# hey-yahei/Quantization.MXNet

Hardware: AMD Instinct MI355X
Metric: images/sec int8-sim MobileNet1.0 (per-layer W8A8, online input quant) (higher is better)
Workload: dtype f32

## Files before the change

quantization/mxnet_amd/csrc/fq_core.hip:

```cpp
#include "fq_common.h"

namespace fqi {

thread_local char g_err[512] = "";

int fail(int code, const char* fmt, ...) {
  va_list ap;
  va_start(ap, fmt);
  vsnprintf(g_err, sizeof(g_err), fmt, ap);
  va_end(ap);
  return code;
}

bool g_prof_on = false;
std::mutex g_prof_mu;
std::vector<ProfRec> g_prof;

void prof_push(const ProfRec& r) {
  std::lock_guard<std::mutex> lk(g_prof_mu);
  g_prof.push_back(r);
}

int num_cu() {
  constexpr int kMaxDev = 64;
  static int cache[kMaxDev] = {0};
  int dev = 0;
  if (hipGetDevice(&dev) != hipSuccess || dev < 0 || dev >= kMaxDev) return 256;
  if (cache[dev] == 0) {
    hipDeviceProp_t prop;
    int cu = 0;
    if (hipGetDeviceProperties(&prop, dev) == hipSuccess) cu = prop.multiProcessorCount;
    cache[dev] = cu > 0 ? cu : 256;
  }
  return cache[dev];
}

int max_lds_bytes() {
  constexpr int kMaxDev = 64;
  static int cache[kMaxDev] = {0};
  int dev = 0;
  if (hipGetDevice(&dev) != hipSuccess || dev < 0 || dev >= kMaxDev) return 160 * 1024;
  if (cache[dev] == 0) {
    int v = 0;
    if (hipDeviceGetAttribute(&v, hipDeviceAttributeMaxSharedMemoryPerBlock, dev) != hipSuccess || v <= 0) v = 160 * 1024;
    cache[dev] = v;
  }
  return cache[dev];
}

int env_int(const char* name, int dflt) {
  const char* e = getenv(name);
  return (e && *e) ? atoi(e) : dflt;
}

constexpr int kPolNtLoad_ = 1, kPolNtStore_ = 2, kPolReverse_ = 4;
int stream_policy(int kernel_id, int64_t numel) {
  static const int ov_stat = env_int("FQ_POLICY_STAT", -1);
  static const int ov_on = env_int("FQ_POLICY_ONLINE", -1);
  static const int ov_off = env_int("FQ_POLICY_OFFLINE", -1);
  static const int64_t big = (int64_t)env_int("FQ_POLICY_BIG_MB", 160) * 1000000;
  const bool is_big = numel * (int64_t)sizeof(float) >= big;
  switch (kernel_id) {
    case FQ_KERNEL_STAT:
      return ov_stat >= 0 ? ov_stat : 0;
    case FQ_KERNEL_APPLY_ONLINE:
      if (ov_on >= 0) return ov_on;
      return is_big ? (kPolReverse_ | kPolNtLoad_ | kPolNtStore_) : kPolReverse_;
    default:
      if (ov_off >= 0) return ov_off;
      return is_big ? (kPolNtLoad_ | kPolNtStore_) : 0;
  }
}

}

using namespace fqi;

extern "C" {

const char* fq_last_error(void) { return g_err; }
int fq_version(void) { return 102; }
#ifndef FQ_BUILD_ID
#define FQ_BUILD_ID "0000000000000000000000000000000000000000"
#endif
const char* fq_build_id(void) {
  static const char id[] = "FQ_BUILD_ID=" FQ_BUILD_ID;
  return id + 12;
}

int fq_device_info(char* arch, int arch_len, int* compute_units, int* wavefront) {
  int dev = 0;
  FQ_HIP(hipGetDevice(&dev));
  hipDeviceProp_t prop;
  FQ_HIP(hipGetDeviceProperties(&prop, dev));
  if (arch != nullptr && arch_len > 0) {
    strncpy(arch, prop.gcnArchName, (size_t)arch_len - 1);
    arch[arch_len - 1] = 0;
  }
  if (compute_units) *compute_units = prop.multiProcessorCount;
  if (wavefront) *wavefront = prop.warpSize;
  return FQ_OK;
}

int fq_profile_enable(int on) {
  g_prof_on = on != 0;
  return FQ_OK;
}

int fq_profile_reset(void) {
  std::lock_guard<std::mutex> lk(g_prof_mu);
  for (auto& r : g_prof) {
    (void)hipEventDestroy(r.a);
    (void)hipEventDestroy(r.b);
  }
  g_prof.clear();
  return FQ_OK;
}

int fq_profile_read_moved(int kernel_id, double* total_moved_bytes) {
  FQ_REQUIRE(kernel_id >= 0 && kernel_id < FQ_KERNEL_COUNT, "fq_profile_read_moved: bad kernel id %d", kernel_id);
  FQ_REQUIRE(total_moved_bytes, "fq_profile_read_moved: null pointer");
  std::lock_guard<std::mutex> lk(g_prof_mu);
  double moved = 0.0;
  for (auto& r : g_prof)
    if (r.kid == kernel_id) moved += r.moved;
  *total_moved_bytes = moved;
  return FQ_OK;
}

int fq_profile_read(int kernel_id, double* total_ms, int64_t* launches, double* total_bytes) {
  FQ_REQUIRE(kernel_id >= 0 && kernel_id < FQ_KERNEL_COUNT, "fq_profile_read: bad kernel id %d", kernel_id);
  FQ_REQUIRE(total_ms && launches && total_bytes, "fq_profile_read: null pointer");
  std::lock_guard<std::mutex> lk(g_prof_mu);
  double ms = 0.0, bytes = 0.0;
  int64_t cnt = 0;
  for (auto& r : g_prof) {
    if (r.kid != kernel_id) continue;
    FQ_HIP(hipEventSynchronize(r.b));
    float t = 0.f;
    FQ_HIP(hipEventElapsedTime(&t, r.a, r.b));
    ms += t;
    bytes += r.bytes;
    ++cnt;
  }
  *total_ms = ms;
  *launches = cnt;
  *total_bytes = bytes;
  return FQ_OK;
}

}

namespace {
__global__ void spin_kernel(unsigned long long* __restrict__ t, unsigned long long ticks) {
  const unsigned long long t0 = wall_clock64();
  unsigned long long t1 = t0;
  while (t1 - t0 < ticks) t1 = wall_clock64();
  if (threadIdx.x == 0) {
    t[0] = t0;
    t[1] = t1;
  }
}
}

extern "C" {

int fq_profile_calibrate(void* scratch, int repeats, double* pair_ms, double* null_kernel_ms, fqStream_t stream) {
  FQ_REQUIRE(scratch && pair_ms && null_kernel_ms && repeats > 0 && repeats <= 4096, "fq_profile_calibrate: bad arguments");
  hipStream_t st = (hipStream_t)stream;
  std::vector<hipEvent_t> ev((size_t)repeats * 2 + 2);
  for (auto& e : ev) FQ_HIP(hipEventCreate(&e));
  for (int i = 0; i < repeats; ++i) {
    FQ_HIP(hipEventRecord(ev[2 * i], st));
    hipLaunchKernelGGL(fill_kernel, dim3(1), dim3(64), 0, st, (float*)scratch, (int64_t)1, 0.0f);
    FQ_HIP(hipEventRecord(ev[2 * i + 1], st));
  }
  FQ_HIP(hipEventRecord(ev[2 * repeats], st));
  for (int i = 0; i < repeats; ++i)
    hipLaunchKernelGGL(fill_kernel, dim3(1), dim3(64), 0, st, (float*)scratch, (int64_t)1, 0.0f);
  FQ_HIP(hipEventRecord(ev[2 * repeats + 1], st));
  FQ_HIP(hipEventSynchronize(ev.back()));
  std::vector<float> ts;
  for (int i = 0; i < repeats; ++i) {
    float t = 0.f;
    FQ_HIP(hipEventElapsedTime(&t, ev[2 * i], ev[2 * i + 1]));
    ts.push_back(t);
  }
  float all = 0.f;
  FQ_HIP(hipEventElapsedTime(&all, ev[2 * repeats], ev[2 * repeats + 1]));
  for (auto& e : ev) (void)hipEventDestroy(e);
  std::sort(ts.begin(), ts.end());
  *pair_ms = ts[ts.size() / 2];
  *null_kernel_ms = (double)all / repeats;
  return FQ_OK;
}

int fq_profile_launch_overhead(void* scratch, int repeats, double spin_us, double* overhead_ms, double* spin_ms,
                               fqStream_t stream) {
  FQ_REQUIRE(scratch && overhead_ms && spin_ms && repeats > 0 && repeats <= 4096 && spin_us > 0 && spin_us < 1e5,
             "fq_profile_launch_overhead: bad arguments");
  hipStream_t st = (hipStream_t)stream;
  int dev = 0, khz = 0;
  FQ_HIP(hipGetDevice(&dev));
  FQ_HIP(hipDeviceGetAttribute(&khz, hipDeviceAttributeWallClockRate, dev));
  FQ_REQUIRE(khz > 0, "fq_profile_launch_overhead: the device reports no wall clock rate");
  const unsigned long long ticks = (unsigned long long)(spin_us * 1e-3 * khz);
  std::vector<hipEvent_t> ev((size_t)repeats * 2 + 2);
  for (auto& e : ev) FQ_HIP(hipEventCreate(&e));
  unsigned long long* t = (unsigned long long*)scratch;
  for (int i = 0; i < repeats; ++i) {
    FQ_HIP(hipEventRecord(ev[2 * i], st));
    hipLaunchKernelGGL(spin_kernel, dim3(1), dim3(64), 0, st, t + 2 * i, ticks);
    FQ_HIP(hipEventRecord(ev[2 * i + 1], st));
  }
  FQ_HIP(hipEventRecord(ev[2 * repeats], st));
  for (int i = 0; i < repeats; ++i) hipLaunchKernelGGL(spin_kernel, dim3(1), dim3(64), 0, st, t + 2 * i, ticks);
  FQ_HIP(hipEventRecord(ev[2 * repeats + 1], st));
  FQ_LAUNCH_CHECK();
  FQ_HIP(hipStreamSynchronize(st));
  std::vector<unsigned long long> host((size_t)repeats * 2);
  FQ_HIP(hipMemcpy(host.data(), t, host.size() * sizeof(unsigned long long), hipMemcpyDeviceToHost));
  std::vector<double> pair, own;
  for (int i = 0; i < repeats; ++i) {
    float el = 0.f;
    FQ_HIP(hipEventElapsedTime(&el, ev[2 * i], ev[2 * i + 1]));
    pair.push_back((double)el);
    own.push_back((double)(host[2 * i + 1] - host[2 * i]) / (double)khz);
  }
  float all = 0.f;
  FQ_HIP(hipEventElapsedTime(&all, ev[2 * repeats], ev[2 * repeats + 1]));
  for (auto& e : ev) (void)hipEventDestroy(e);
  std::sort(pair.begin(), pair.end());
  std::sort(own.begin(), own.end());
  *overhead_ms = pair[pair.size() / 2] - (double)all / repeats;
  *spin_ms = own[own.size() / 2];
  return FQ_OK;
}

}
```

quantization/mxnet_amd/csrc/fq_front_layout.h:

```cpp
#pragma once

#include <cstddef>
#include <cstdint>

#if defined(__HIPCC__)
#define FQ_FL_FN __host__ __device__ __forceinline__
#else
#define FQ_FL_FN inline
#endif

namespace fqi {

constexpr int kFrontRows = 8;
constexpr int kFrontBandBytes = 32768;
constexpr int kStatLdsPerCU = 160 * 1024, kStatLdsMax = 120 * 1024;

struct FrontLayout {
  int js;
  int pl;
};

FQ_FL_FN FrontLayout front_layout(int q, int rows) {
  FrontLayout l;
  l.js = rows * q + ((8 - rows * q) & 15);
  l.pl = 4 * l.js + 16;
  return l;
}

FQ_FL_FN int front_slot(FrontLayout l, int p) { return (p & 3) * l.js + (p >> 2); }

FQ_FL_FN int front_byte(FrontLayout l, int c, int p) { return (((c >> 2) * l.pl + front_slot(l, p)) << 2) + (c & 3); }

inline size_t front_band_bytes(int q, int rows, int cin) { return (size_t)((cin + 3) / 4) * front_layout(q, rows).pl * 4; }

FQ_FL_FN int front_channel(int c0, int wave, int segs, int seg) { return c0 + wave * segs + seg; }

FQ_FL_FN int mfma_row_pixel(int i32) { return 16 * ((i32 >> 2) & 1) + 4 * (i32 >> 3) + (i32 & 3); }

inline int stat_wg_per_cu(size_t lds, int cap) {
  const int by_lds = (int)((size_t)kStatLdsPerCU / (lds + 1024));
  return by_lds > cap ? cap : (by_lds < 1 ? 1 : by_lds);
}

inline int front_rows_pick(int64_t n, int64_t h, int64_t w, int cin, size_t lds_fixed, int num_cu, int wg_cap, int forced = 0) {
  const int q = (int)(w / 4);
  int rmax = (int)(kFrontBandBytes / (32 * w));
  rmax = rmax > kFrontRows ? kFrontRows : rmax;
  rmax = rmax > h ? (int)h : rmax;
  while (rmax >= 1 && lds_fixed + front_band_bytes(q, rmax, cin) > (size_t)kStatLdsMax) --rmax;
  if (rmax < 1) return 0;
  if (forced > 0) return forced < rmax ? forced : rmax;
  {
    int r2 = rmax;
    while (r2 >= 1 && stat_wg_per_cu(lds_fixed + front_band_bytes(q, r2, cin), wg_cap) < 2) --r2;
    if (r2 >= 1) rmax = r2;
  }
  double best = 1e30;
  int best_r = rmax;
  bool best_whole = false;
  for (int r = rmax; r >= 1; --r) {
    const int64_t wgs = n * ((h + r - 1) / r);
    const int64_t slots = (int64_t)num_cu * stat_wg_per_cu(lds_fixed + front_band_bytes(q, r, cin), wg_cap);
    const int64_t grid = wgs < slots ? wgs : slots, rounds = (wgs + grid - 1) / grid;
    const double cost = (double)(rounds * ((grid + num_cu - 1) / num_cu) * (r + 2));
    const bool whole = (r * w) % 32 == 0;
    if (cost < best - 1e-9 || (cost < best + 1e-9 && whole && !best_whole)) {
      best = cost;
      best_r = r;
      best_whole = whole;
    }
  }
  return best_r;
}

}
```

quantization/mxnet_amd/csrc/fq_pwdw.hip:

```cpp
#include "fq_pw.h"

#include "fq_front_layout.h"

#include <climits>

namespace {

struct PwDwGeom {
  int Cin, KTS, Cout, H, W, Ho, Wo;
  int strips, ctg, bands, RB;
  int zoff, pitch;
  int vw;
  FastDiv qv;
};

constexpr int kRowSlack = 8;

template <int KT, int S> struct PwDwRing {
  static constexpr int NB = S == 1 ? 2 : (KT <= 2 ? 3 : 4);
  static constexpr int NR = 2;
};

template <int KT, int CW, int S, int LZ, int FAST, int CODES, int NS = 0>
__global__ __launch_bounds__(512) void pwdw_kernel(
// ... 141 lines not shown
      } else {
        return fq_pack4<false>(a, b, c, d, q1, ubias1, nn_xor1);
      }
    };
    constexpr int NO = S == 1 ? 16 : 8;
    float sumA[CW][NO], sumB[S == 1 ? CW : 1][NO];
#pragma unroll
    for (int j = 0; j < CW; ++j)
#pragma unroll
      for (int k = 0; k < NO; ++k) {
        sumA[j][k] = 0.0f;
        if (S == 1) sumB[j][k] = 0.0f;
      }
    QParams qc = q2;
    if (FAST) qc.hi = fminf(q2.hi, top);

    auto row = [&](int t, auto ph_c) __attribute__((always_inline)) {
      constexpr int PH = decltype(ph_c)::value;
      const bool row_ok = t >= 0 && t < g.H;
      v4i afrag[KT];
      if constexpr (CODES) {
        issue_row(t + NR - 1, crow[(PH + NR - 1) % NR]);
        FQ_PIN();
#pragma unroll
        for (int kt = 0; kt < KT; ++kt) afrag[kt] = crow[PH % NR][kt];
      } else {
#pragma unroll
        for (int kt = 0; kt < KT; ++kt) {
          const int qn = kt + NB - 1;
          issue(t + qn / KT, qn % KT, raw[(PH * KT + kt + NB - 1) % NB]);
          FQ_PIN();
          float (&mine)[16] = raw[(PH * KT + kt) % NB];
          v4i f;
#pragma unroll
          for (int d = 0; d < 4; ++d)
            f[d] = pack_x(mine[4 * d + 0], mine[4 * d + 1], mine[4 * d + 2], mine[4 * d + 3]);
          asm volatile("" : "+v"(f[0]), "+v"(f[1]), "+v"(f[2]), "+v"(f[3]));
          afrag[kt] = f;
          FQ_PIN();
        }
      }
      const int r_emit = S == 1 ? t - 1 : (t - 1) >> 1;
      const bool emits = (S == 1 || (t & 1)) && r_emit >= ro0 && r_emit < ro1;
      float* rbuf = rowbuf + (r_emit & 1) * rb_stride;
#pragma unroll
      for (int j = 0; j < CW; ++j) {
        const int ct = cgi * CW + j;
        const float* kc = ldsK + (ct * 32 + i32) * 13;
        auto finish_store = [&](const float (&sum)[NO]) __attribute__((always_inline)) {
          if (!emits) return;
          float* dst = rbuf + (ct * 32 + i32) * g.pitch + obase;
          float mrow = 0.0f;
          const float b2 = kDwLds ? kc[9] : k_b2[j], bsc2 = kDwLds ? kc[10] : k_bsc2[j], bsh2 = kDwLds ? kc[11] : k_bsh2[j];
#pragma unroll
          for (int k = 0; k < NO; ++k) {
            float o;
            if (FAST == 0) {
              o = dw_finish<kEpiRuntime>(sum[k], has_b2, b2, has_bn2, bsc2, bsh2, act2);
            } else {
              o = sum[k] * bsc2;
              o = o + bsh2;
              o = __builtin_amdgcn_fmed3f(o, 0.0f, top);
            }
            if constexpr (NS != 0) {
              const bool is_out = k == 0 ? h == 1 : (k == NO - 1 ? h == 0 : (LZ == 0 || k > LZ || h == 1));
              mrow = fmaxf(mrow, is_out ? fabsf(o) : 0.0f);
            } else if (S == 1 && k == 0) {
              if (h == 1) dst[k] = o;
            } else if (k == NO - 1) {
              if (h == 0) dst[k] = o;
            } else {
              dst[k] = o;
            }
          }
          if constexpr (NS != 0) m = fmaxf(m, mrow);
        };
        if (!row_ok) {
          if (S == 1) {
            finish_store(sumA[j]);
#pragma unroll
            for (int k = 0; k < 16; ++k) {
              sumA[j][k] = sumB[j][k];
              sumB[j][k] = 0.0f;
            }
          } else if (t & 1) {
            finish_store(sumA[j]);
#pragma unroll
            for (int c = 0; c < 8; ++c) sumA[j][c] = 0.0f;
          }
          FQ_PIN();
          continue;
        }
        float e[18];
        float cf[NS ? 18 : 1];
        {
          v16i acc = {0, 0, 0, 0, 0, 0, 0, 0, 0, 0, 0, 0, 0, 0, 0, 0};
          int wl = lane;
          asm volatile("" : "+v"(wl));
#pragma unroll
          for (int kt = 0; kt < KT; ++kt)
            acc = __builtin_amdgcn_mfma_i32_32x32x32_i8(afrag[kt], ldsW[((ct * KT + kt) << 6) + wl], acc, 0, 0, 0);
#pragma unroll
          for (int k = 0; k < 16; ++k) {
            float v = (float)(acc[k] + k_zs[j]) * k_sxw[j];
            if (FAST == 0) {
              if (has_b1) v = v + k_b1[j];
              if (has_bn1) {
                v = v * k_bsc1[j];
                v = v + k_bsh1[j];
              }
              v = act_rt(v, act1);
              const float code = NN ? truncf(fast_quot(fq_clip(v, q2), fq2) + 0.49999997f) : fq_code(v, q2);
              e[k + 1] = code * q2.scale;
              if constexpr (NS != 0) cf[k + 1] = code;
            } else {
              v = v * k_bsc1[j];
              v = v + k_bsh1[j];
              const float code = NN ? truncf(fast_quot(fq_clip(v, qc), fq2) + 0.49999997f)
                                    : fq_code(act_rt(v, relu6 ? FQ_ACT_RELU6 : FQ_ACT_RELU), q2);
              e[k + 1] = code * q2.scale;
              if constexpr (NS != 0) cf[k + 1] = code;
            }
          }
          if constexpr (NS != 0) {
            const auto sc = __builtin_amdgcn_permlane32_swap(__float_as_uint(cf[1]), __float_as_uint(cf[16]), false, false);
            cf[0] = __uint_as_float(sc[0]);
            cf[17] = __uint_as_float(sc[1]);
            auto pk4 = [&](float a, float b, float c, float d) __attribute__((always_inline)) {
              if constexpr (NN) {
                unsigned u = __builtin_amdgcn_cvt_pk_u8_f32(a, 0, 0u);
                u = __builtin_amdgcn_cvt_pk_u8_f32(b, 1, u);
                u = __builtin_amdgcn_cvt_pk_u8_f32(c, 2, u);
                return (int)__builtin_amdgcn_cvt_pk_u8_f32(d, 3, u);
              } else {
                return (int)(((unsigned)(int)a & 255u) | (((unsigned)(int)b & 255u) << 8) | (((unsigned)(int)c & 255u) << 16) |
                             ((unsigned)(int)d << 24));
              }
            };
            typedef int v3i __attribute__((ext_vector_type(3)));
            typedef unsigned v3u __attribute__((ext_vector_type(3)));
            v3i d3;
            int dx;
            if (ns_par2) {
              d3 = (v3i){pk4(cf[4], cf[5], cf[6], cf[7]), pk4(cf[8], cf[9], cf[10], cf[11]), pk4(cf[12], cf[13], cf[14], cf[15])};
              dx = pk4(h ? cf[0] : cf[2], h ? cf[1] : cf[3], cf[2], cf[3]);
            } else {
              d3 = (v3i){pk4(cf[2], cf[3], cf[4], cf[5]), pk4(cf[6], cf[7], cf[8], cf[9]), pk4(cf[10], cf[11], cf[12], cf[13])};
              dx = pk4(cf[14], cf[15], cf[16], cf[17]);
            }
            const unsigned rowb = (unsigned)((ct * 32 + i32) * HW + t * g.W);
            if (ns_ok3) {
              __builtin_amdgcn_raw_buffer_store_b96(__builtin_bit_cast(v3u, d3), rsy, (int)(rowb + (unsigned)ns_col3), 0, 0);
              asm volatile("s_nop 1" : : "v"(d3));
            }
            if (ns_okx) {
              if (ns_x4) __builtin_amdgcn_raw_buffer_store_b32((unsigned)dx, rsy, (int)(rowb + (unsigned)ns_colx), 0, 0);
              else __builtin_amdgcn_raw_buffer_store_b16((unsigned short)dx, rsy, (int)(rowb + (unsigned)ns_colx), 0, 0);
            }
          }
          e[1 + (LZ & 15)] = zero_left ? 0.0f : e[1 + (LZ & 15)];
          if (S == 1) e[16] = zero_right ? 0.0f : e[16];
          const auto sw = __builtin_amdgcn_permlane32_swap(__float_as_uint(e[1]), __float_as_uint(e[16]), false, false);
          e[0] = __uint_as_float(sw[0]);
          e[17] = __uint_as_float(sw[1]);
        }
        float w[9];
        if (!kDwLds) {
#pragma unroll
          for (int t = 0; t < 9; ++t) w[t] = k_w[j][t];
        }
        if (S == 1) {
          w[6] = kc[6]; w[7] = kc[7]; w[8] = kc[8];
#pragma unroll
          for (int k = 0; k < 16; ++k) {
            float a = sumA[j][k];
            a = fmaf(w[6], e[k], a);
            a = fmaf(w[7], e[k + 1], a);
            a = fmaf(w[8], e[k + 2], a);
            sumA[j][k] = a;
          }
          finish_store(sumA[j]);
          w[0] = kc[0]; w[1] = kc[1]; w[2] = kc[2]; w[3] = kc[3]; w[4] = kc[4]; w[5] = kc[5];
#pragma unroll
          for (int k = 0; k < 16; ++k) {
            float b = sumB[j][k];
            b = fmaf(w[3], e[k], b);
            b = fmaf(w[4], e[k + 1], b);
            b = fmaf(w[5], e[k + 2], b);
            float c = 0.0f;
            c = fmaf(w[0], e[k], c);
            c = fmaf(w[1], e[k + 1], c);
            c = fmaf(w[2], e[k + 2], c);
            sumA[j][k] = b;
            sumB[j][k] = c;
          }
        } else {
          if (t & 1) {
#pragma unroll
            for (int c = 0; c < 8; ++c) {
              float a = sumA[j][c];
              a = fmaf(w[6], e[2 * c + 1], a);
              a = fmaf(w[7], e[2 * c + 2], a);
              a = fmaf(w[8], e[2 * c + 3], a);
              sumA[j][c] = a;
            }
            finish_store(sumA[j]);
#pragma unroll
            for (int c = 0; c < 8; ++c) {
              float a = 0.0f;
              a = fmaf(w[0], e[2 * c + 1], a);
              a = fmaf(w[1], e[2 * c + 2], a);
              a = fmaf(w[2], e[2 * c + 3], a);
              sumA[j][c] = a;
            }
          } else {
#pragma unroll
            for (int c = 0; c < 8; ++c) {
              float a = sumA[j][c];
              a = fmaf(w[3], e[2 * c + 1], a);
              a = fmaf(w[4], e[2 * c + 2], a);
              a = fmaf(w[5], e[2 * c + 3], a);
              sumA[j][c] = a;
            }
          }
        }
        FQ_PIN();
      }
      if (NS == 0 && emits) {
        __syncthreads();
        const unsigned per_row = g.qv.d;
        const int vecs = g.Cout * (int)per_row;
        float* yr = yb + (int64_t)r_emit * g.Wo;
        for (int idx = threadIdx.x; idx < vecs; idx += blockDim.x) {
          const unsigned c = fast_div((unsigned)idx, g.qv), qd = (unsigned)idx - c * per_row;
          if (g.vw == 4) {
            const float* src = rbuf + c * g.pitch + 4 * qd;
            const f4 v = (f4){src[0], src[1], src[2], src[3]};
            m = fmaxf(fmaxf(m, fmaxf(fabsf(v.x), fabsf(v.y))), fmaxf(fabsf(v.z), fabsf(v.w)));
            *reinterpret_cast<f4*>(yr + (int64_t)c * g.Ho * g.Wo + 4 * qd) = v;
          } else if (g.vw == 2) {
            const float* src = rbuf + c * g.pitch + 2 * qd;
            const float2 v = make_float2(src[0], src[1]);
            m = fmaxf(m, fmaxf(fabsf(v.x), fabsf(v.y)));
            *reinterpret_cast<float2*>(yr + (int64_t)c * g.Ho * g.Wo + 2 * qd) = v;
          } else {
            const float v = rbuf[c * g.pitch + qd];
            m = fmaxf(m, fabsf(v));
            yr[(int64_t)c * g.Ho * g.Wo + qd] = v;
          }
        }
      }
    };
    constexpr int U = CODES ? NR : ((KT % NB == 0) ? 1 : ((2 * KT) % NB == 0 ? 2 : NB));
    static_assert(U <= 3, "the row loop below unrolls at most three phases");
    using std::integral_constant;
    for (int t = t_first; t <= t_last; t += U) {
      row(t, integral_constant<int, 0>{});
      if (U > 1 && t + 1 <= t_last) row(t + 1, integral_constant<int, 1 % U>{});
      if (U > 2 && t + 2 <= t_last) row(t + 2, integral_constant<int, 2 % U>{});
    }
  };
  using std::false_type;
  using std::true_type;
  if (fq_nonneg(q1) && fq_nonneg(q2) && fq1.ok && fq2.ok) body(true_type{});
  else body(false_type{});

  if (stat_out != nullptr) {
    m = wave_max_nonneg(m);
    __syncthreads();
    if (lane == 0) red[wave] = m;
    __syncthreads();
    if (threadIdx.x == 0) {
      float mm = 0.0f;
      for (int w = 0; w < (int)(blockDim.x >> 6); ++w) mm = fmaxf(mm, red[w]);
      if (__float_as_uint(mm) != 0u) FQ_STAT_FLUSH_MAX(reinterpret_cast<unsigned*>(stat_out) + smp, __float_as_uint(mm));
    }
  }
}

__device__ __forceinline__ void buf_st_v4i(fq_rsrc r, unsigned voff, v4i v) {
  typedef unsigned v4u __attribute__((ext_vector_type(4)));
  __builtin_amdgcn_raw_buffer_store_b128(__builtin_bit_cast(v4u, v), r, (int)voff, 0, 0);
  asm volatile("s_nop 1" : : "v"(v));
}

struct PwStatGeom {
  int Cin, KTS, Cout, CT, HW;
  int64_t cols, tiles;
  int zoff;
  int table;
  FastDiv hw;
};

struct PwFrontArgs {
  const int8_t* codes;
  const float *w, *bias, *bn_scale, *bn_shift;
  const float *in_stat, *in_thr;
  float levels;
  int act;
  int H, W, Q, segs, R, bands;
  FrontLayout lay;
};

template <int KT, int FEPI = -1, bool FSIGNED = false>
__global__ __launch_bounds__(kBlock, 3) void pw_stat_kernel(
    const float* __restrict__ x, const int8_t* __restrict__ wfrag, const float* __restrict__ wscale,
    const int* __restrict__ wsum, const float* __restrict__ bias, PwStatGeom g, const float* __restrict__ in_stat, int n,
    const float* __restrict__ in_thr, float levels, int lo_neg, float eps, float* __restrict__ cur_max_out,
    const float* __restrict__ bn_scale, const float* __restrict__ bn_shift, int act, float* __restrict__ stat_out,
    int8_t* __restrict__ x_codes_out, PwFrontArgs fa) {
  constexpr bool FRONT = FEPI >= 0;
  static_assert(!FRONT || KT <= 4, "the front layer is built for up to four 32-channel slabs");
  extern __shared__ __attribute__((aligned(16))) unsigned char pst_smem[];
  v4i* ldsW = reinterpret_cast<v4i*>(pst_smem);
  int* c_zs = reinterpret_cast<int*>(pst_smem + (size_t)g.CT * KT * 1024);
  float* c_k = reinterpret_cast<float*>(c_zs + g.CT * 32);
  int* accs = reinterpret_cast<int*>(c_k + 4 * g.CT * 32);
  float* dwk = reinterpret_cast<float*>(accs + 4 * g.CT * 128);
  unsigned char* zbuf = reinterpret_cast<unsigned char*>(dwk + g.Cin * 12);
  const int lane = threadIdx.x & 63, wave = threadIdx.x >> 6;
  const int h = lane >> 5, i32 = lane & 31;
  const unsigned HW = (unsigned)g.HW, cols = (unsigned)g.cols;
  const int64_t nwaves = (int64_t)gridDim.x * 4, wid = (int64_t)blockIdx.x * 4 + wave;
  const int64_t n_bands = FRONT ? (int64_t)(g.cols / g.HW) * fa.bands : 0;
  const int64_t t_begin = FRONT ? n_bands * blockIdx.x / gridDim.x : g.tiles * wid / nwaves;
  const int64_t t_end = FRONT ? n_bands * (blockIdx.x + 1) / gridDim.x : g.tiles * (wid + 1) / nwaves;
  const int pl = mfma_row_pixel(i32);
  int* my = accs + (size_t)wave * g.CT * 128;
  constexpr int kSlots = 8;
  __shared__ unsigned k_stat[kSlots];
  if (threadIdx.x < kSlots) k_stat[threadIdx.x] = 0u;
  unsigned s_base;
  if constexpr (FRONT) {
    s_base = (unsigned)((t_begin < n_bands ? t_begin : n_bands - 1) / fa.bands);
  } else {
    const int64_t t0 = g.tiles * ((int64_t)blockIdx.x * 4) / nwaves;
    const unsigned j0 = (unsigned)(t0 < g.tiles ? t0 : g.tiles - 1) * 32u;
    s_base = fast_div(j0 < cols ? j0 : cols - 1, g.hw);
  }

  struct Pix { unsigned smp, p; };
  auto pix_of = [&](int64_t t) __attribute__((always_inline)) {
    unsigned j = (unsigned)t * 32u + (unsigned)pl;
    j = j < cols ? j : cols - 1;
    Pix r;
    r.smp = fast_div(j, g.hw);
    r.p = j - r.smp * HW;
    return r;
  };
  constexpr int NB = 3;
  const fq_rsrc rs = make_rsrc(x, (int64_t)(cols / HW) * g.Cin * HW * 4);
  auto issue = [&](int64_t t, int kt, float (&v)[16]) __attribute__((always_inline)) {
    if (t >= t_end) return;
    const Pix px = pix_of(t);
    const bool ok = kt * 32 + 16 * h < g.Cin;
    const unsigned vo = ok ? (unsigned)(((px.smp * (unsigned)g.Cin + 16u * h) * HW + px.p) * 4u) : 0x80000000u;
    const unsigned so = (unsigned)kt * 32u * HW * 4u;
#pragma unroll
    for (int i = 0; i < 16; ++i) v[i] = buf_ld_f32(rs, vo, so + (unsigned)i * HW * 4u);
  };
  float raw[NB][16];
#pragma unroll
  for (int b2 = 0; b2 < NB; ++b2)
#pragma unroll
    for (int i = 0; i < 16; ++i) raw[b2][i] = 0.0f;
  if constexpr (!FRONT) {
#pragma unroll
    for (int qq = 0; qq < NB - 1; ++qq) issue(t_begin + qq / KT, qq % KT, raw[qq]);
  }
  FQ_PIN();
  float fscale = 0.0f;
  if constexpr (FRONT) fscale = input_threshold(fa.in_stat, n, fa.in_thr, nullptr, false) / fa.levels;
  const float max_ = input_threshold(in_stat, n, in_thr, cur_max_out, blockIdx.x == 0);
  const QParams q = make_qparams(max_, levels, lo_neg != 0, eps);
  const int ubias = 128 - g.zoff;
  const unsigned nn_xor = fq_nonneg_xor(ubias);
  const bool wr_codes = x_codes_out != nullptr;
  const fq_rsrc rcodes = make_rsrc(x_codes_out, wr_codes ? (int64_t)(cols / HW) * 2 * KT * HW * 16 : 0);
  for (int idx = threadIdx.x; idx < g.CT * KT * 64; idx += kBlock) {
    const int f = idx >> 6, ct = f / KT, kt = f - ct * KT;
    ldsW[idx] = *reinterpret_cast<const v4i*>(wfrag + (((int64_t)ct * g.KTS + kt) << 10) + ((idx & 63) << 4));
  }
  const int nchs = g.CT * 32;
  for (int i = threadIdx.x; i < nchs; i += kBlock) {
    const bool okc = i < g.Cout;
    c_zs[i] = okc ? g.zoff * wsum[i] : 0;
    c_k[i] = okc ? wscale[i] : 0.0f;
    c_k[nchs + i] = (okc && bias != nullptr) ? bias[i] : 0.0f;
    c_k[2 * nchs + i] = (okc && bn_scale != nullptr) ? bn_scale[i] : 1.0f;
    c_k[3 * nchs + i] = (okc && bn_scale != nullptr) ? bn_shift[i] : 0.0f;
  }
  if constexpr (FRONT)
    for (int i = threadIdx.x; i < g.Cin; i += kBlock) {
#pragma unroll
      for (int t = 0; t < 9; ++t) dwk[i * 12 + t] = fa.w[i * 9 + t];
      dwk[i * 12 + 9] = fa.bias != nullptr ? fa.bias[i] : 0.0f;
      dwk[i * 12 + 10] = fa.bn_scale != nullptr ? fa.bn_scale[i] : 1.0f;
      dwk[i * 12 + 11] = fa.bn_scale != nullptr ? fa.bn_shift[i] : 0.0f;
    }
  auto reset = [&]() __attribute__((always_inline)) {
    for (int ct = 0; ct < g.CT; ++ct) {
      my[ct * 128 + lane] = INT_MIN;
      my[ct * 128 + 64 + lane] = INT_MAX;
    }
  };
  reset();
  __syncthreads();
  const bool has_bn = bn_scale != nullptr;
  auto flush = [&](unsigned smp) __attribute__((always_inline)) {
    float m = 0.0f;
    for (int ct = 0; ct < g.CT; ++ct) {
      const int c = ct * 32 + i32;
      int hi = my[ct * 128 + lane], lo = my[ct * 128 + 64 + lane];
      const int ohi = __shfl_xor(hi, 32, 64), olo = __shfl_xor(lo, 32, 64);
      hi = hi > ohi ? hi : ohi;
      lo = lo < olo ? lo : olo;
      if (c < g.Cout && hi >= lo) {
        hi += c_zs[c];
        lo += c_zs[c];
        const float sxw = q.scale * c_k[c];
        const float bch = c_k[nchs + c];
        const float bsc = c_k[2 * nchs + c], bsh = c_k[3 * nchs + c];
        auto f = [&](int a) {
          float v = (float)a * sxw;
          if (bias != nullptr) v = v + bch;
          if (has_bn) {
            v = v * bsc;
            v = v + bsh;
          }
          return fabsf(act_rt(v, act));
        };
        m = fmaxf(m, fmaxf(f(hi), f(lo)));
      }
    }
    m = wave_max_nonneg(m);
    if (lane == 0 && __float_as_uint(m) != 0u) {
      const unsigned slot = smp - s_base;
      if (g.table && slot < (unsigned)kSlots) atomicMax(&k_stat[slot], __float_as_uint(m));
      else FQ_STAT_FLUSH_MAX(reinterpret_cast<unsigned*>(stat_out) + smp, __float_as_uint(m));
    }
    reset();
  };
  v4i afrag[KT];
  const FastQuot fqx = make_fast_quot(q.denom);
  auto quant = [&](int kt, const float (&v)[16], auto nn_c) __attribute__((always_inline)) {
    v4i f;
#pragma unroll
    for (int d = 0; d < 4; ++d) {
      if constexpr (decltype(nn_c)::value) {
        unsigned u = 0u;
#pragma unroll
        for (int b = 0; b < 4; ++b) {
          int r;
          const float Q = fast_quot(fq_clip(v[4 * d + b], q), fqx);
          asm("v_cvt_rpi_i32_f32 %0, %1" : "=v"(r) : "v"(Q));
          u |= (unsigned)r << (8 * b);
        }
        f[d] = (int)(u ^ nn_xor);
      } else {
        f[d] = fq_pack4<false>(v[4 * d + 0], v[4 * d + 1], v[4 * d + 2], v[4 * d + 3], q, ubias, nn_xor);
      }
    }
    asm volatile("" : "+v"(f[0]), "+v"(f[1]), "+v"(f[2]), "+v"(f[3]));
    afrag[kt] = f;
  };
  auto reduce_tile = [&](int plo, int phi) __attribute__((always_inline)) {
    const bool whole = plo <= 0 && phi >= 32;
#pragma unroll 1
    for (int ct = 0; ct < g.CT; ++ct) {
      v16i acc = {0, 0, 0, 0, 0, 0, 0, 0, 0, 0, 0, 0, 0, 0, 0, 0};
#pragma unroll
      for (int kt = 0; kt < KT; ++kt)
        acc = __builtin_amdgcn_mfma_i32_32x32x32_i8(afrag[kt], ldsW[((ct * KT + kt) << 6) + lane], acc, 0, 0, 0);
      int hi = INT_MIN, lo = INT_MAX;
      if (whole) {
#pragma unroll
        for (int k = 0; k < 16; k += 2) {
          hi = max(max(acc[k], acc[k + 1]), hi);
          lo = min(min(acc[k], acc[k + 1]), lo);
        }
      } else {
#pragma unroll
        for (int k = 0; k < 16; ++k) {
          const int p = 16 * h + k;
          const bool in = p >= plo && p < phi;
          hi = in && acc[k] > hi ? acc[k] : hi;
          lo = in && acc[k] < lo ? acc[k] : lo;
        }
      }
      atomicMax(&my[ct * 128 + lane], hi);
      atomicMin(&my[ct * 128 + 64 + lane], lo);
    }
  };
  unsigned cur = FRONT ? s_base : fast_div((unsigned)((t_begin < g.tiles ? t_begin : g.tiles - 1) * 32), g.hw);
  auto run_tile = [&](int64_t t, auto ph_c, auto nn_c) __attribute__((always_inline)) {
    constexpr int PH = decltype(ph_c)::value;
    const Pix px = pix_of(t);
    const unsigned cvo = ((px.smp * (unsigned)(2 * KT) + (unsigned)h) * HW + px.p) * 16u;
#pragma unroll
    for (int kt = 0; kt < KT; ++kt) {
      const int qn = kt + NB - 1;
      issue(t + qn / KT, qn % KT, raw[(PH * KT + kt + NB - 1) % NB]);
      FQ_PIN();
      quant(kt, raw[(PH * KT + kt) % NB], nn_c);
      if (wr_codes) buf_st_v4i(rcodes, cvo + (unsigned)(2 * kt) * HW * 16u, afrag[kt]);
      FQ_PIN();
    }
    const unsigned j0 = (unsigned)t * 32u, j1 = j0 + 31u < cols ? j0 + 31u : cols - 1;
    const unsigned s0 = fast_div(j0, g.hw), s1 = fast_div(j1, g.hw);
    if (s0 != cur) {
      flush(cur);
      cur = s0;
    }
    if (s0 == s1) {
      reduce_tile(0, 32);
    } else {
      const int pb = (int)(s1 * HW - j0);
      reduce_tile(0, pb);
      flush(cur);
      cur = s1;
      reduce_tile(pb, 32);
    }
    FQ_PIN();
  };
  auto run_all = [&](auto nn_c) __attribute__((always_inline)) {
    constexpr int U = (KT % NB == 0) ? 1 : NB;
    using std::integral_constant;
    for (int64_t t = t_begin; t < t_end; t += U) {
      run_tile(t, integral_constant<int, 0>{}, nn_c);
      if (U > 1 && t + 1 < t_end) run_tile(t + 1, integral_constant<int, 1 % U>{}, nn_c);
      if (U > 2 && t + 2 < t_end) run_tile(t + 2, integral_constant<int, 2 % U>{}, nn_c);
      if (U > 3 && t + 3 < t_end) run_tile(t + 3, integral_constant<int, 3 % U>{}, nn_c);
    }
  };
  auto run_front = [&](auto nn_c) __attribute__((always_inline)) {
    constexpr bool NN = decltype(nn_c)::value;
    constexpr int FE = FRONT ? FEPI : kEpiRuntime;
    const int Q = fa.Q, W = fa.W, H = fa.H;
    const int seg = lane / Q, pos = lane - seg * Q;
    const bool first = pos == 0, last = pos == Q - 1;
    const bool has_fb = fa.bias != nullptr, has_fbn = fa.bn_scale != nullptr;
    QParams qc = q;
    if (NN && FE != kEpiRuntime) qc.hi = FE == kEpiBnRelu6 ? fminf(q.hi, 6.0f) : q.hi;
    const unsigned* xc32 = reinterpret_cast<const unsigned*>(fa.codes);
    const int z4 = stored_zero4(ubias);
    const v4i zero_frag = (v4i){z4, z4, z4, z4};
    auto deq = [&](unsigned wd, int b) __attribute__((always_inline)) {
      const int code = FSIGNED ? (int)(int8_t)(wd >> (8 * b)) : (int)((wd >> (8 * b)) & 255u);
      return (float)code * fscale;
    };
    for (int64_t bt = t_begin; bt < t_end; ++bt) {
      const unsigned smp = (unsigned)(bt / fa.bands);
      const int r0 = (int)(bt - (int64_t)smp * fa.bands) * fa.R;
      const int Rb = H - r0 < fa.R ? H - r0 : fa.R;
      if (smp != cur) {
        flush(cur);
        cur = smp;
      }
      for (int c0 = 0; c0 < g.Cin; c0 += 4 * fa.segs) {
        const int c = front_channel(c0, wave, fa.segs, seg);
        const bool c_ok = seg < fa.segs && c < g.Cin;
        const int cc = c_ok ? c : 0;
        const float* kc = dwk + cc * 12;
        const float w00 = kc[0], w01 = kc[1], w02 = kc[2], w10 = kc[3], w11 = kc[4], w12 = kc[5], w20 = kc[6], w21 = kc[7],
                    w22 = kc[8], bch = kc[9], bsc = kc[10], bsh = kc[11];
        const unsigned* src = xc32 + ((int64_t)(smp * (unsigned)g.Cin + (unsigned)cc) * H) * Q + pos;
        unsigned raw_c[kFrontRows + 2];
#pragma unroll
        for (int k = 0; k < kFrontRows + 2; ++k) {
          const int t = r0 - 1 + k, tc = t < 0 ? 0 : (t > H - 1 ? H - 1 : t);
          raw_c[k] = src[tc * Q] & ((t >= 0 && t < H) ? 0xFFFFFFFFu : 0u);
        }
        auto zcode = [&](float acc) __attribute__((always_inline)) {
          if constexpr (NN) {
            const float v = FE == kEpiRuntime ? dw_finish<kEpiRuntime>(acc, has_fb, bch, has_fbn, bsc, bsh, fa.act)
                                              : dw_finish<FE, false>(acc, false, 0.0f, true, bsc, bsh, 0);
            int r;
            const float Qv = fast_quot(fq_clip(v, qc), fqx);
            asm("v_cvt_rpi_i32_f32 %0, %1" : "=v"(r) : "v"(Qv));
            return (unsigned)r ^ (nn_xor & 255u);
          } else {
            const float v = dw_finish<FE>(acc, has_fb, bch, has_fbn, bsc, bsh, fa.act);
            return (unsigned)(fq_code_int(v, q) + ubias) ^ 0x80u;
          }
        };
        float a[6] = {0.f, 0.f, 0.f, 0.f, 0.f, 0.f}, b[6] = {0.f, 0.f, 0.f, 0.f, 0.f, 0.f};
        unsigned dst = (unsigned)front_byte(fa.lay, cc, 4 * pos);
        const unsigned jstep = (unsigned)(front_byte(fa.lay, 0, 1) - front_byte(fa.lay, 0, 0));
        const unsigned rstep = (unsigned)(front_byte(fa.lay, 0, 4 * Q) - front_byte(fa.lay, 0, 0));
#pragma unroll
        for (int k = 0; k < kFrontRows + 2; ++k) {
          if (k <= Rb + 1) {
            float cv[6];
#pragma unroll
            for (int j = 0; j < 4; ++j) cv[j + 1] = deq(raw_c[k], j);
            const float lp = lane_prev(cv[4]), ln = lane_next(cv[1]);
            cv[0] = first ? 0.0f : lp;
            cv[5] = last ? 0.0f : ln;
            if (k >= 2) {
#pragma unroll
              for (int j = 0; j < 4; ++j) {
                const unsigned code = zcode(dw_taps(w00, w01, w02, w10, w11, w12, w20, w21, w22, a[j], a[j + 1], a[j + 2], b[j],
                                                    b[j + 1], b[j + 2], cv[j], cv[j + 1], cv[j + 2]));
                if (c_ok) zbuf[dst + j * jstep] = (unsigned char)code;
              }
              dst += rstep;
              asm volatile("" : "+v"(dst));
            }
#pragma unroll
            for (int j = 0; j < 6; ++j) {
              a[j] = b[j];
              b[j] = cv[j];
            }
          }
        }
      }
      __syncthreads();
      const int npix = Rb * W, ntile = (npix + 31) >> 5;
      for (int tl = wave; tl < ntile; tl += 4) {
        int pp = tl * 32 + pl;
        pp = pp < npix ? pp : npix - 1;
        const unsigned* zp = reinterpret_cast<const unsigned*>(zbuf + front_byte(fa.lay, g.Cin <= 16 ? 0 : 16 * h, pp));
#pragma unroll
        for (int kt = 0; kt < KT; ++kt) {
          v4i f;
#pragma unroll
          for (int u = 0; u < 4; ++u) f[u] = (int)zp[(8 * kt + u) * fa.lay.pl];
          if (KT == 1 && g.Cin <= 16 && h == 1) f = zero_frag;
          if (wr_codes)
            buf_st_v4i(rcodes, ((smp * (unsigned)(2 * KT) + (unsigned)(2 * kt + h)) * HW + (unsigned)(r0 * W + pp)) * 16u, f);
          afrag[kt] = f;
        }
        const int valid = npix - tl * 32;
        reduce_tile(0, valid < 32 ? valid : 32);
      }
      __syncthreads();
    }
  };
  if constexpr (FRONT) {
    if (fq_nonneg(q) && fqx.ok) run_front(std::true_type{});
    else run_front(std::false_type{});
  } else {
    if (fq_nonneg(q) && fqx.ok) run_all(std::true_type{});
    else run_all(std::false_type{});
  }
  if (t_begin < t_end) flush(cur);
  __syncthreads();
  if (threadIdx.x < kSlots && k_stat[threadIdx.x] != 0u && s_base + threadIdx.x < cols / HW)
    FQ_STAT_FLUSH_MAX(reinterpret_cast<unsigned*>(stat_out) + s_base + threadIdx.x, k_stat[threadIdx.x]);
}

__global__ void fast_quotient_kernel(const float* __restrict__ c, int64_t n, const float* __restrict__ d, float* __restrict__ out,
                                     int* __restrict__ ok_out) {
  const FastQuot f = make_fast_quot(d[0]);
  const double rden = 1.0 / (double)d[0];
  const int64_t i = (int64_t)blockIdx.x * blockDim.x + threadIdx.x;
  if (i == 0) ok_out[0] = f.ok ? 1 : 0;
  if (i < n) out[i] = f.ok ? fast_quot(c[i], f) : ieee_div_by(c[i], rden);
}

struct PwDwPlan {
  int kt, cw, lz, strips, ctg, bands, rb, pitch, threads;
  size_t lds;
  bool ok;
};

PwDwPlan pwdw_plan(int64_t n, int64_t cin, int64_t cout, int64_t h, int64_t w, int stride) {
  PwDwPlan p;
  memset(&p, 0, sizeof(p));
  if (n <= 0 || cin <= 0 || cout <= 0 || h < 3 || w < 8 || (stride != 1 && stride != 2)) return p;
  if (cout % 32 != 0 || (stride == 2 && (w % 2 != 0 || h % 2 != 0))) return p;
  const int kt = (int)((cin + 31) / 32), ct = (int)(cout / 32);
  if (!(kt == 1 || kt == 2 || kt == 4 || kt == 8)) return p;
  const int wo = (int)((w - 1) / stride + 1), ho = (int)((h - 1) / stride + 1);
  p.kt = kt;
  p.cw = ct % 2 == 0 ? 2 : 1;
  p.strips = (int)((w + 29) / 30);
  p.lz = (stride == 1 && p.strips == 1) ? (int)(30 - w) : 0;
  if (!(p.lz == 0 || p.lz == 2)) return p;
  p.ctg = ct / p.cw;
  p.threads = 64 * p.strips * p.ctg;
  if (p.threads > 512) return p;
  const int reach = stride == 1 ? (int)w + 2 + p.lz : 15 * p.strips + 1;
  p.pitch = (reach > wo ? reach : wo) + p.lz;
  p.pitch |= 1;
  p.lds = (size_t)ct * kt * 1024 + 2 * ((size_t)cout * p.pitch + kRowSlack) * 4 + kRowSlack * 4 + (stride == 1 ? (size_t)cout * 13 * 4 : 0);
  if (p.lds + 10 * 1024 > (size_t)max_lds_bytes()) return p;
  const char* rb_e = getenv("FQ_PWDW_RB");
  const int rb_env = rb_e != nullptr ? atoi(rb_e) : 0;
  {
    const int waves = p.threads / 64;
    int occ = (int)((160 * 1024) / (p.lds + 512));
    const int by_regs = 8 / waves > 0 ? 8 / waves : 1;
    occ = occ < by_regs ? occ : by_regs;
    occ = occ < 1 ? 1 : occ;
    const double slots = (double)num_cu() * occ;
    double best = 1e30;
    int best_rb = ho;
    for (int b = 1; b <= ho; ++b) {
      const int rb = (ho + b - 1) / b, bands = (ho + rb - 1) / rb;
      const double wgs = (double)n * bands, rounds = ceil(wgs / slots), fill = wgs < slots ? wgs / slots : 1.0;
      const double cost = rounds * (stride * rb + 2) / fill;
      if (cost < best - 1e-9) {
        best = cost;
        best_rb = rb;
      }
    }
    p.rb = rb_env > 0 ? (rb_env < ho ? rb_env : ho) : best_rb;
  }
  p.bands = (ho + p.rb - 1) / p.rb;
  if (n * cin * h * w * 4 >= (1ll << 32) || n * cout * ho * wo >= (1ll << 31)) return p;
  p.ok = true;
  return p;
}

}

namespace fqi {

static size_t pw_stat_lds(int kt, int ct) { return (size_t)ct * kt * 1024 + 5 * (size_t)ct * 32 * 4 + 4 * (size_t)ct * 128 * 4; }

bool pw_stat_shape_ok(int64_t n, int64_t cin, int64_t cout, int64_t hw) {
  if (n <= 0 || cin <= 0 || cout <= 0 || hw < 32 || hw >= (1ll << 30) || n * hw >= (1ll << 31) - 512) return false;
  const int kt = (int)((cin + 31) / 32), ct = (int)((cout + 31) / 32);
  if (!(kt == 1 || kt == 2 || kt == 4 || kt == 8) || cin % 16 != 0) return false;
  return pw_stat_lds(kt, ct) <= (size_t)kStatLdsMax && n * cin * hw * 4 < (1ll << 32);
}

constexpr int kFrontWgCap = 4;

static int pw_front_rows(int64_t n, int64_t cin, int64_t cout, int64_t h, int64_t w) {
  const char* e = getenv("FQ_PWSTAT_FRONT_ROWS");
  static const int wg_env = env_int("FQ_PWSTAT_WG_PER_CU", 0);
  const size_t fixed = pw_stat_lds((int)((cin + 31) / 32), (int)((cout + 31) / 32)) + (size_t)cin * 12 * 4;
  return front_rows_pick(n, h, w, (int)cin, fixed, num_cu(), wg_env > 0 ? wg_env : kFrontWgCap, e != nullptr ? atoi(e) : 0);
}

bool pw_stat_front_shape_ok(int64_t n, int64_t cin, int64_t cout, int64_t h, int64_t w) {
  if (h < 1 || w < 4 || w % 4 != 0 || w / 4 > 64 || !(cin == 16 || cin == 32 || cin == 64 || cin == 128) ||
      !pw_stat_shape_ok(n, cin, cout, h * w))
    return false;
  return pw_front_rows(n, cin, cout, h, w) >= 1 && n * cin * ((w / 4 + 61) / 62) < (1ll << 31) - 1024;
}

int pw_stat_launch(const PwCall& c) {
  const int kt = (int)((c.cin + 31) / 32), ct = (int)((c.cout + 31) / 32);
  size_t lds = pw_stat_lds(kt, ct);
  PwFrontArgs fa = {};
  if (c.front != nullptr) {
    const PwFront& f = *c.front;
    fa.codes = static_cast<const int8_t*>(f.codes);
    fa.w = f.w; fa.bias = f.bias; fa.bn_scale = f.bn_scale; fa.bn_shift = f.bn_shift;
    fa.in_stat = f.in_stat; fa.in_thr = f.in_thr; fa.levels = f.levels; fa.act = f.act;
    fa.H = (int)f.h; fa.W = (int)f.wdt; fa.Q = fa.W / 4; fa.segs = 64 / fa.Q;
    fa.R = pw_front_rows(c.n, c.cin, c.cout, f.h, f.wdt);
    FQ_REQUIRE(fa.R >= 1, "fq_pwconv_i8_stat: no band of the front layer fits the LDS");
    fa.bands = (fa.H + fa.R - 1) / fa.R;
    fa.lay = front_layout(fa.Q, fa.R);
    lds += (size_t)c.cin * 12 * 4 + front_band_bytes(fa.Q, fa.R, (int)c.cin);
  }
  PwStatGeom g;
  g.Cin = (int)c.cin; g.KTS = (int)(c.cin_pad / 32); g.Cout = (int)c.cout; g.CT = ct; g.HW = (int)c.hw;
  g.cols = c.n * c.hw; g.tiles = (g.cols + 31) / 32; g.zoff = c.zoff;
  g.hw = fast_div_for((unsigned)c.hw);
  if (int rc = pw_zero_stat(c)) return rc;
  int per_cu = stat_wg_per_cu(lds, c.front != nullptr ? kFrontWgCap : 3);
  static const int wg_env = env_int("FQ_PWSTAT_WG_PER_CU", 0);
  if (wg_env > 0) per_cu = wg_env;
  int64_t grid = (int64_t)num_cu() * per_cu;
  const int64_t need = c.front != nullptr ? c.n * fa.bands : (g.tiles + 3) / 4;
  if (grid > need) grid = need;
  static const int table_env = env_int("FQ_PWSTAT_TABLE", -1);
  g.table = table_env >= 0 ? table_env : (g.tiles < grid * 4 * 10 ? 1 : 0);
#define FQ_PST_GO(KT_)                                                                                                     \
  case KT_: {                                                                                                              \
    static const bool attr_ok = hipFuncSetAttribute(reinterpret_cast<const void*>(&pw_stat_kernel<KT_>),                   \
                                                    hipFuncAttributeMaxDynamicSharedMemorySize, 120 * 1024) == hipSuccess; \
    FQ_REQUIRE(attr_ok, "fq_pwconv_i8_stat: cannot raise the dynamic LDS limit");                                          \
    hipLaunchKernelGGL((pw_stat_kernel<KT_>), dim3((unsigned)grid), dim3(kBlock), lds, c.st, c.x, c.wcodes, c.wscale,       \
                       (const int*)c.wsum, c.bias, g, c.in_stat, (int)c.n, c.in_thr, c.levels, c.lo_neg, kEps,              \
                       c.out_current_max, c.bn_scale, c.bn_shift, c.act, c.stat_out, (int8_t*)c.x_codes_out, fa);          \
  } break;
#define FQ_PST_FRONT(KT_, EPI_, SG_)                                                                                       \
  {                                                                                                                        \
    static const bool attr_ok = hipFuncSetAttribute(reinterpret_cast<const void*>(&pw_stat_kernel<KT_, EPI_, SG_>),        \
                                                    hipFuncAttributeMaxDynamicSharedMemorySize, 120 * 1024) == hipSuccess; \
    FQ_REQUIRE(attr_ok, "fq_pwconv_i8_stat: cannot raise the dynamic LDS limit");                                          \
    hipLaunchKernelGGL((pw_stat_kernel<KT_, EPI_, SG_>), dim3((unsigned)grid), dim3(kBlock), lds, c.st, c.x, c.wcodes,     \
                       c.wscale, (const int*)c.wsum, c.bias, g, c.in_stat, (int)c.n, c.in_thr, c.levels, c.lo_neg, kEps,   \
                       c.out_current_max, c.bn_scale, c.bn_shift, c.act, c.stat_out, (int8_t*)c.x_codes_out, fa);          \
  }
#define FQ_PST_FRONT_S(KT_, EPI_)                                                                                          \
  {                                                                                                                        \
    if (c.front->is_signed) FQ_PST_FRONT(KT_, EPI_, true) else FQ_PST_FRONT(KT_, EPI_, false)                              \
  }
#define FQ_PST_FRONT_E(KT_)                                                                                                \
  {                                                                                                                        \
    if (c.front->epi == kEpiBnRelu) FQ_PST_FRONT_S(KT_, kEpiBnRelu)                                                        \
    else if (c.front->epi == kEpiBnRelu6) FQ_PST_FRONT_S(KT_, kEpiBnRelu6)                                                 \
    else FQ_PST_FRONT_S(KT_, kEpiRuntime)                                                                                  \
  }
  if (c.front != nullptr) {
    FQ_REQUIRE(kt == 1 || kt == 2 || kt == 4, "fq_pwconv_i8_stat: a front layer needs cin <= 128");
    if (kt == 1) FQ_PST_FRONT_E(1) else if (kt == 2) FQ_PST_FRONT_E(2) else FQ_PST_FRONT_E(4)
  } else {
    switch (kt) {
      FQ_PST_GO(1) FQ_PST_GO(2) FQ_PST_GO(4) FQ_PST_GO(8)
      default: return fail(FQ_ERR_INVALID, "fq_pwconv_i8_stat: K / 32 = %d is not instantiated", kt);
    }
  }
#undef FQ_PST_FRONT_E
#undef FQ_PST_FRONT_S
#undef FQ_PST_FRONT
#undef FQ_PST_GO
  FQ_LAUNCH_CHECK();
  return FQ_OK;
}

}

using namespace fqi;

extern "C" {

int fq_debug_fast_quotient(const float* c, int64_t n, const float* d, float* out, int* took_fast_path, fqStream_t stream) {
  FQ_REQUIRE(c && d && out && took_fast_path && n > 0, "fq_debug_fast_quotient: null pointer");
  hipLaunchKernelGGL(fast_quotient_kernel, dim3((unsigned)((n + 255) / 256)), dim3(256), 0, (hipStream_t)stream, c, n, d, out,
                     took_fast_path);
  FQ_LAUNCH_CHECK();
  return FQ_OK;
}

int fq_pwdw_fused_supported(int64_t n, int64_t cin, int64_t cout, int64_t h, int64_t w, int stride, int stat_mode) {
  if (stat_mode != 0 && !(stride == 1 && w % 4 == 0 && n * cout * h * w < (1ll << 31))) return 0;
  return pwdw_plan(n, cin, cout, h, w, stride).ok ? 1 : 0;
}

}

static int pwdw_fused_impl(const float* x, const int8_t* wcodes, const float* wscale, const int32_t* wsum, const float* pw_bias,
                           int64_t n, int64_t cin, int64_t cin_pad, int64_t cout_pad, int64_t cout, int64_t h, int64_t w,
                           const float* in_stat, const float* in_thr, int in_width, unsigned in_flags, const float* pw_bn_scale,
                           const float* pw_bn_shift, int pw_act, const float* mid_stat, const float* mid_thr, int mid_width,
                           unsigned mid_flags, float* mid_current_max, const float* dw_w, const float* dw_bias, int dw_stride,
                           const float* dw_bn_scale, const float* dw_bn_shift, int dw_act, float* y, void* mid_codes_out,
                           float* stat_out, const void* x_codes, fqStream_t stream) {
  const bool ns = mid_codes_out != nullptr;
  FQ_REQUIRE((x || x_codes) && wcodes && wscale && wsum && dw_w && (y || ns), "fq_pwdw_fused: null pointer");
  if (ns) {
    FQ_REQUIRE(y == nullptr && stat_out && x_codes && dw_stride == 1 && aligned16(mid_codes_out),
               "fq_pwdw_fused: the statistic mode (mid_codes_out) wants y == NULL, stat_out, x_codes, stride 1 and a 16-byte aligned buffer");
    FQ_REQUIRE(w % 4 == 0 && mid_width <= 8 && ((mid_flags & FQ_ACT_SIGNED) || !(mid_flags & FQ_ACT_LO_NEG_MAX)) &&
                   n * cout * h * w < (1ll << 31) && cout * h * w < (1ll << 31) - 64,
               "fq_pwdw_fused: statistic mode: shape or quantiser not taken (rows of whole dwords, codes that fit a byte): see "
               "fq_pwdw_fused_supported(..., stat_mode = 1)");
  }
  FQ_REQUIRE(in_stat != nullptr || in_thr != nullptr, "fq_pwdw_fused: give in_stat (online) or in_thr (offline)");
  FQ_REQUIRE(mid_stat != nullptr || mid_thr != nullptr, "fq_pwdw_fused: give mid_stat (the per-sample maxima of the pointwise "
             "output, from fq_pwconv_i8_stat) or mid_thr (a stored threshold)");
  FQ_REQUIRE(in_width >= 2 && in_width <= 8, "fq_pwdw_fused: input width %d does not fit int8 codes", in_width);
  FQ_REQUIRE(mid_width >= 2 && mid_width <= 16, "fq_pwdw_fused: bad width %d of the depthwise input", mid_width);
  FQ_REQUIRE(!((in_flags | mid_flags) & (FQ_ACT_NO_ABS | FQ_ACT_NO_EPS)), "fq_pwdw_fused: unsupported activation flags");
  FQ_REQUIRE((pw_bn_scale == nullptr) == (pw_bn_shift == nullptr) && (dw_bn_scale == nullptr) == (dw_bn_shift == nullptr),
             "fq_pwdw_fused: a BatchNorm's scale and shift go together");
  FQ_REQUIRE(cin_pad >= cin && cin_pad % 64 == 0 && cout_pad >= cout && cout_pad % 32 == 0,
             "fq_pwdw_fused: cin_pad / cout_pad must be those of fq_weight_codes");
  const bool prezeroed = (dw_act & FQ_STAT_PREZEROED) != 0;
  dw_act &= ~FQ_STAT_PREZEROED;
  FQ_REQUIRE(pw_act >= FQ_ACT_NONE && pw_act <= FQ_ACT_RELU6 && dw_act >= FQ_ACT_NONE && dw_act <= FQ_ACT_RELU6,
             "fq_pwdw_fused: unknown activation");
  FQ_REQUIRE(aligned16(wcodes) && (x_codes ? aligned16(x_codes) : aligned16(x)) && (ns || aligned16(y)),
             "fq_pwdw_fused: x (x_codes when given), wcodes and y must be 16-byte aligned");
  const PwDwPlan p = pwdw_plan(n, cin, cout, h, w, dw_stride);
  FQ_REQUIRE(p.ok, "fq_pwdw_fused: shape not taken (n=%lld cin=%lld cout=%lld %lldx%lld stride %d): see fq_pwdw_fused_supported",
             (long long)n, (long long)cin, (long long)cout, (long long)h, (long long)w, dw_stride);
  hipStream_t st = (hipStream_t)stream;
  const int64_t ho = (h - 1) / dw_stride + 1, wo = (w - 1) / dw_stride + 1;
  if (stat_out && !prezeroed) FQ_HIP(hipMemsetAsync(stat_out, 0, n * sizeof(float), st));
  PwDwGeom g;
  g.Cin = (int)cin; g.KTS = (int)(cin_pad / 32); g.Cout = (int)cout; g.H = (int)h; g.W = (int)w; g.Ho = (int)ho; g.Wo = (int)wo;
  g.strips = p.strips; g.ctg = p.ctg; g.bands = p.bands; g.RB = p.rb;
  g.zoff = (in_flags & FQ_ACT_SIGNED) ? 0 : 128;
  g.pitch = p.pitch;
  g.vw = wo % 4 == 0 ? 4 : (wo % 2 == 0 ? 2 : 1);
  g.qv = fast_div_for((unsigned)(wo / g.vw));
  const int8_t* wfrag = wcodes + cout_pad * cin_pad;
  const float levels1 = act_levels(in_width, in_flags), levels2 = act_levels(mid_width, mid_flags);
  const int lo1 = (in_flags & FQ_ACT_LO_NEG_MAX) ? 1 : 0, lo2 = (mid_flags & FQ_ACT_LO_NEG_MAX) ? 1 : 0;
  int fast = 0;
  if (!pw_bias && !dw_bias && pw_bn_scale && dw_bn_scale && !lo1 && !lo2 && pw_act == dw_act &&
      (pw_act == FQ_ACT_RELU || pw_act == FQ_ACT_RELU6))
    fast = 1;
  static const int no_fast = env_int("FQ_PWDW_NO_FAST", 0);
  if (no_fast) fast = 0;
  const double in_elems = (double)n * cin * h * w, mid_elems = (double)n * cout * h * w, out_elems = (double)n * cout * ho * wo;
  const double in_moved = x_codes ? 32.0 * p.kt * (double)n * h * w : 4.0 * in_elems;
  const double out_moved = ns ? (double)n * cout * w * (h + 2.0 * (p.bands - 1)) : 4.0 * out_elems;
  ProfScope prof(FQ_KERNEL_DWCONV, 4.0 * (mid_elems + out_elems), st, in_moved + out_moved);
  const int8_t* xc = static_cast<const int8_t*>(x_codes);
  const unsigned grid = (unsigned)(n * p.bands);
  const size_t lds = ns ? (size_t)(cout / 32) * p.kt * 1024 + (size_t)cout * 13 * 4 : p.lds;
  float* const y_arg = ns ? static_cast<float*>(mid_codes_out) : y;
#define FQ_PWDW_GO(KT_, CW_, S_, LZ_, F_, C_, NS_)                                                                          \
  {                                                                                                                        \
    static const bool attr_ok =                                                                                            \
        hipFuncSetAttribute(reinterpret_cast<const void*>(&pwdw_kernel<KT_, CW_, S_, LZ_, F_, C_, NS_>),                    \
                            hipFuncAttributeMaxDynamicSharedMemorySize, 150 * 1024) == hipSuccess;                         \
    FQ_REQUIRE(attr_ok, "fq_pwdw_fused: cannot raise the dynamic LDS limit");                                              \
    hipLaunchKernelGGL((pwdw_kernel<KT_, CW_, S_, LZ_, F_, C_, NS_>), dim3(grid), dim3((unsigned)p.threads), lds, st, x,    \
                       xc, wfrag, wscale, (const int*)wsum, pw_bias, g, in_stat, (int)n, in_thr, levels1, lo1, kEps,        \
                       pw_bn_scale, pw_bn_shift, pw_act, mid_stat, mid_thr, levels2, lo2, mid_current_max, dw_w, dw_bias,   \
                       dw_bn_scale, dw_bn_shift, dw_act, y_arg, stat_out);                                                 \
  }
#define FQ_PWDW_C(KT_, CW_, S_, LZ_, F_)                                                                                    \
  {                                                                                                                        \
    if (xc != nullptr) FQ_PWDW_GO(KT_, CW_, S_, LZ_, F_, 1, 0) else FQ_PWDW_GO(KT_, CW_, S_, LZ_, F_, 0, 0)                 \
  }
#define FQ_PWDW_F(KT_, CW_, S_, LZ_)                                                                                        \
  {                                                                                                                        \
    if (fast == 1) FQ_PWDW_C(KT_, CW_, S_, LZ_, 1) else FQ_PWDW_C(KT_, CW_, S_, LZ_, 0)                                     \
  }
#define FQ_PWDW_N(KT_, CW_, LZ_)                                                                                            \
  {                                                                                                                        \
    if (fast == 1) FQ_PWDW_GO(KT_, CW_, 1, LZ_, 1, 1, 1) else FQ_PWDW_GO(KT_, CW_, 1, LZ_, 0, 1, 1)                         \
  }
#define FQ_PWDW_S(KT_, CW_)                                                                                                 \
  {                                                                                                                        \
    if (dw_stride == 2) FQ_PWDW_F(KT_, CW_, 2, 0)                                                                          \
    else if (ns) {                                                                                                         \
      if (p.lz == 0) FQ_PWDW_N(KT_, CW_, 0) else FQ_PWDW_N(KT_, CW_, 2)                                                    \
    } else if (p.lz == 0) FQ_PWDW_F(KT_, CW_, 1, 0) else FQ_PWDW_F(KT_, CW_, 1, 2)                                          \
  }
#define FQ_PWDW_K(KT_)                                                                                                      \
  case KT_:                                                                                                                \
    if (p.cw == 2) FQ_PWDW_S(KT_, 2) else FQ_PWDW_S(KT_, 1)                                                                \
    break;
  switch (p.kt) {
    FQ_PWDW_K(1) FQ_PWDW_K(2) FQ_PWDW_K(4) FQ_PWDW_K(8)
    default: break;
  }
#undef FQ_PWDW_K
#undef FQ_PWDW_S
#undef FQ_PWDW_N
#undef FQ_PWDW_F
#undef FQ_PWDW_C
#undef FQ_PWDW_GO
  FQ_LAUNCH_CHECK();
  return FQ_OK;
}

extern "C" {

int fq_pwdw_fused(const float* x, const int8_t* wcodes, const float* wscale, const int32_t* wsum, const float* pw_bias,
                  int64_t n, int64_t cin, int64_t cin_pad, int64_t cout_pad, int64_t cout, int64_t h, int64_t w,
                  const float* in_stat, const float* in_thr, int in_width, unsigned in_flags, const float* pw_bn_scale,
                  const float* pw_bn_shift, int pw_act, const float* mid_stat, const float* mid_thr, int mid_width,
                  unsigned mid_flags, float* mid_current_max, const float* dw_w, const float* dw_bias, int dw_stride,
                  const float* dw_bn_scale, const float* dw_bn_shift, int dw_act, float* y, float* stat_out,
                  const void* x_codes, fqStream_t stream, void* mid_codes_out) {
  return pwdw_fused_impl(x, wcodes, wscale, wsum, pw_bias, n, cin, cin_pad, cout_pad, cout, h, w, in_stat, in_thr, in_width,
                         in_flags, pw_bn_scale, pw_bn_shift, pw_act, mid_stat, mid_thr, mid_width, mid_flags, mid_current_max,
                         dw_w, dw_bias, dw_stride, dw_bn_scale, dw_bn_shift, dw_act, y, mid_codes_out, stat_out, x_codes, stream);
}

}
```

quantization/mxnet_amd/ops.py:

```python
import ctypes
import threading

import numpy as np
import torch

from . import _lib
from ._lib import FakeQuantError

__all__ = ["comm_unique_id", "comm_init", "comm_world", "comm_allreduce", "comm_destroy", "add_act_stat", "bn_act_maxpool_stat", "stat_rows_sum", "mean_from_sums", "fake_quant_online_prestat", "bn_act_stat", "stem_conv3x3s2", "stem_conv_s2", "stem_conv_supported", "eval_counters", "dense_i8_eval", "gemm_i8_codes", "global_avg_pool_stat", "dwconv3x3", "dwconv3x3_c16", "weight_codes", "pwconv_i8", "pwconv_strided_supported", "weight_codes_3x3", "weight_slices_3x3", "conv3x3_i8", "Codes16", "batch_mean_rows", "batch_mean_gathered", "ste_forward", "absmax_per_sample", "batch_mean", "fake_quant_online", "fake_quant_offline", "weight_fake_quant",
           "wino_weight_fake_quant", "ema_update", "global_max", "histogram_accumulate", "hist_to_float",
           "kl_search", "quantize_codes", "dequantize", "qconv_kind", "qconv_weights", "qconv_workspace", "qconv2d",
           "batches_in_flight", "in_flight", "winograd_matrices", "device_info", "act_flags"]

_WS = {}


def _lib_():
    return _lib.LIB


_DEVICE_TLS = threading.local()


def _stream(t):
# ... 346 lines not shown
    n, inner = _n_inner(a)
    y = torch.empty_like(a) if out is None else _check(out, "out")
    stat, zflag = _stat_target(n, a.device, want_stat)
    if hist is not None:
        check_call(_lib_().fq_add_act_stat_hist(_ptr(a), _ptr(b), _ptr(y), n, inner, _ACTS[act] | zflag, _ptr(stat),
                                                *_hist_args(hist, want_stat), _stream(a)))
        return y, stat
    check_call(_lib_().fq_add_act_stat(_ptr(a), _ptr(b), _ptr(y), n, inner, _ACTS[act] | zflag, _ptr(stat), _stream(a)))
    return y, stat


def global_avg_pool_stat(x, want_stat=True):
    _check(x, "x")
    if x.dim() != 4:
        raise ValueError("global_avg_pool_stat wants (N, C, H, W)")
    n, c, h, w = x.shape
    y = torch.empty((n, c, 1, 1), dtype=torch.float32, device=x.device)
    stat, zflag = _stat_target(n, x.device, want_stat)
    check_call(_lib_().fq_global_avg_pool_stat(_ptr(x), _ptr(y), n, c, h * w, int(zflag), _ptr(stat), _stream(x)))
    return y, stat


def gemm_i8_codes(xcodes, wcodes, n, l, zoff):
    require_hip(xcodes.device, "xcodes")
    require_hip(wcodes.device, "wcodes")
    if xcodes.dtype != torch.int8 or wcodes.dtype != torch.int8 or xcodes.dim() != 2 or wcodes.dim() != 2 \
            or xcodes.shape[1] != wcodes.shape[1] or xcodes.shape[0] != n * l:
        raise ValueError("gemm_i8_codes wants xcodes (n*l, K) and wcodes (Cout, K), both int8")
    k, cout = xcodes.shape[1], wcodes.shape[0]
    kp, rp, cp = (k + 31) // 32 * 32, (cout + 31) // 32 * 32, (n * l + 31) // 32 * 32
    xc = torch.zeros((cp, kp), dtype=torch.int8, device=xcodes.device)
    xc[:n * l, :k] = xcodes
    wc = torch.zeros((rp, kp), dtype=torch.int8, device=xcodes.device)
    wc[:cout, :k] = wcodes
    wsum = wcodes.to(torch.int32).sum(dim=1).to(torch.int32).contiguous()
    out = torch.empty((n, cout, l), dtype=torch.int32, device=xcodes.device)
    check_call(_lib_().fq_gemm_i8_codes(xc.data_ptr(), wc.data_ptr(), wsum.data_ptr(), out.data_ptr(), n, l, kp, cout,
                                        int(zoff), _stream(xcodes)))
    return out


_EVAL_WS = {}


def dense_i8_eval(x, wcodes, wscale, wsum, labels, counters, bias=None, in_stat=None, in_thr=None, width=8, flags=0,
                  cur_out=None):
    _check(x, "x")
    _check(wcodes, "wcodes", torch.int8)
    _check(wscale, "wscale")
    _check(wsum, "wsum", torch.int32)
    _check(counters, "counters")
    require_hip(labels.device, "labels")
    for name, t in (("bias", bias), ("in_stat", in_stat), ("in_thr", in_thr), ("cur_out", cur_out)):
        if t is not None:
            _check(t, name)
    n, cin = x.shape[0], x.shape[1]
    cout, cin_pad = wscale.numel(), wcodes.shape[1]
    if x.numel() != n * cin:
        raise ValueError("dense_i8_eval wants (N, Cin) or (N, Cin, 1, 1) activations, got %s" % (tuple(x.shape),))
    if (cin + 63) // 64 * 64 != cin_pad:
        raise ValueError("x has %d channels but the weight codes were made for a row length that pads to %d"
                         % (cin, cin_pad))
    if labels.dim() != 1 or labels.shape[0] != n or labels.dtype != torch.int64:
        raise ValueError("dense_i8_eval wants labels (N,) int64")
    if counters.numel() != 2 + 2 * cout:
        raise ValueError("counters must hold 2 + 2 * %d floats" % cout)
    if in_stat is not None and cur_out is None:
        cur_out = torch.empty(1, dtype=torch.float32, device=x.device)
    nbytes = _lib_().fq_dense_i8_eval_workspace_bytes(n, cout)
    key = (str(x.device), int(nbytes), int(torch.cuda.current_stream(x.device).cuda_stream))
    ews = _EVAL_WS.get(key)
    if ews is None:
        ews = _EVAL_WS[key] = torch.zeros(nbytes // 8 + 1, dtype=torch.int64, device=x.device)
    y = torch.empty((n, cout), dtype=torch.float32, device=x.device)
    ws = torch.empty(_lib_().fq_pwconv_workspace_bytes(n, cin_pad, 1), dtype=torch.uint8, device=x.device)
    lb = labels.contiguous()
    check_call(_lib_().fq_dense_i8_eval(_ptr(x), _ptr(wcodes), _ptr(wscale), _ptr(wsum), _ptr(bias), _ptr(y), n, cin,
                                        cin_pad, cout, _ptr(in_stat), _ptr(in_thr), int(width), int(flags), _ptr(cur_out),
                                        lb.data_ptr(), _ptr(counters), ews.data_ptr(), _ptr(ws), _stream(x)))
    return y


def eval_counters(logits, labels, counters):
    _check(logits, "logits")
    _check(counters, "counters")
    require_hip(labels.device, "labels")
    if logits.dim() != 2 or labels.dim() != 1 or labels.shape[0] != logits.shape[0] or labels.dtype != torch.int64:
        raise ValueError("eval_counters wants logits (N, classes) float32 and labels (N,) int64")
    n, classes = logits.shape
    if counters.numel() != 2 + 2 * classes or not counters.is_contiguous():
        raise ValueError("counters must hold 2 + 2*classes contiguous floats")
    lg = logits if logits.is_contiguous() else logits.contiguous()
    lb = labels if labels.is_contiguous() else labels.contiguous()
    check_call(_lib_().fq_eval_counters(_ptr(lg), lb.data_ptr(), n, classes, _ptr(counters), _stream(logits)))
    return counters


def stem_conv_s2(x, w, bias=None, bn_scale=None, bn_shift=None, act=None, want_stat=True, w_tap_major=None, out_codes=None,
                 pool=False):
    _check(x, "x")
    _check(w, "w")
    if x.dim() != 4 or w.dim() != 4 or w.shape[2] != w.shape[3] or w.shape[2] not in (3, 7) or w.shape[1] != x.shape[1]:
        raise ValueError("stem_conv_s2 wants x (N,C,H,W) and w (Cout,C,K,K), K = 3 or 7; got %s and %s"
                         % (tuple(x.shape), tuple(w.shape)))
    for name, t in (("bias", bias), ("bn_scale", bn_scale), ("bn_shift", bn_shift), ("w_tap_major", w_tap_major)):
        if t is not None:
            _check(t, name)
    act = act or "none"
    if act not in _ACTS:
        raise ValueError("unknown activation %r" % (act,))
    n, cin, h, wd = x.shape
    cout, ks = w.shape[0], w.shape[2]
    pad = ks // 2
    wt = w_tap_major if w_tap_major is not None else w.permute(1, 2, 3, 0).contiguous()
    y = torch.empty((n, cout, (h + 2 * pad - ks) // 2 + 1, (wd + 2 * pad - ks) // 2 + 1), dtype=torch.float32,
                    device=x.device)
    stat, zflag = _stat_target(n, x.device, want_stat)
    if out_codes is not None:
        if ks != 3:
            raise ValueError("the first convolution hands codes over in its 3x3 form only")
        othr = _check(out_codes["thr"], "out_codes['thr']")
        yc = Codes16.empty(tuple(y.shape), x.device, othr, out_codes.get("width", 8), out_codes.get("flags", 0))
        check_call(_lib_().fq_stem_conv3x3s2_c16(_ptr(x), _ptr(wt), _ptr(bias), _ptr(yc.t), n, cin, cout, h, wd, _ptr(bn_scale),
                                                 _ptr(bn_shift), _ACTS[act] | zflag, _ptr(stat), _ptr(othr), int(yc.width),
                                                 int(yc.flags), _stream(x)))
        return yc, stat
    if pool:
        if ks != 7 or not stem_pool_supported(h, wd):
            raise ValueError("the pooled form is built for the 7x7 first convolution on planes whose output rows cut into four "
                             "tiles of at most 32 columns; got K = %d on %d x %d" % (ks, h, wd))
        ho, wo = y.shape[2], y.shape[3]
        yp = torch.empty((n, cout, (ho - 1) // 2 + 1, (wo - 1) // 2 + 1), dtype=torch.float32, device=x.device)
        check_call(_lib_().fq_stem_conv7x7s2_pool(_ptr(x), _ptr(wt), _ptr(bias), _ptr(yp), n, cin, cout, h, wd, _ptr(bn_scale),
                                                  _ptr(bn_shift), _ACTS[act] | zflag, _ptr(stat), _stream(x)))
        return yp, stat
    entry = _lib_().fq_stem_conv3x3s2 if ks == 3 else _lib_().fq_stem_conv7x7s2
    check_call(entry(_ptr(x), _ptr(wt), _ptr(bias), _ptr(y), n, cin, cout, h, wd, _ptr(bn_scale), _ptr(bn_shift),
                     _ACTS[act] | zflag, _ptr(stat), _stream(x)))
    return y, stat


stem_conv3x3s2 = stem_conv_s2


def stem_pool_supported(h, w):
    return bool(_lib_().fq_stem_conv7x7s2_pool_supported(int(h), int(w)))


def stem_conv_supported(cin, cout, kernel, stride, pad):
    k, s, p = tuple(kernel), tuple(stride), tuple(pad)
    return cin == 3 and s == (2, 2) and ((cout == 32 and k == (3, 3) and p == (1, 1)) or
                                         (cout == 64 and k == (7, 7) and p == (3, 3)))


def front_codes_shape(xshape):
    n, c, h, w = (int(v) for v in xshape)
    return (n, c, h * w)


def _check_front_codes(t, name, xshape, device):
    _check(t, name, torch.int8)
    if len(xshape) != 4 or tuple(t.shape) != front_codes_shape(xshape):
        raise ValueError("%s must be int8 %s for a depthwise input %s; got %s"
                         % (name, front_codes_shape(xshape) if len(xshape) == 4 else "(4-d x)", tuple(xshape), tuple(t.shape)))
    if t.device != device:
        raise ValueError("%s lives on %s, x on %s" % (name, t.device, device))
    if t.data_ptr() % 16:
        raise ValueError("%s must be 16-byte aligned" % name)
    return t


def dwconv3x3(x, w, bias=None, stride=1, in_stat=None, in_thr=None, width=8, flags=0, cur_out=None, bn_scale=None,
              bn_shift=None, act=None, want_stat=True, store=True, x_codes_out=None):
    _check(x, "x")
    _check(w, "w")
    if x.dim() != 4 or w.dim() != 4 or tuple(w.shape[1:]) != (1, 3, 3) or w.shape[0] != x.shape[1]:
        raise ValueError("dwconv3x3 wants x (N,C,H,W) and w (C,1,3,3); got %s and %s" % (tuple(x.shape), tuple(w.shape)))
    for name, t in (("bias", bias), ("in_stat", in_stat), ("in_thr", in_thr), ("bn_scale", bn_scale),
                    ("bn_shift", bn_shift), ("cur_out", cur_out)):
        if t is not None:
            _check(t, name)
    n, c, h, wd = x.shape
    ho, wo = (h - 1) // stride + 1, (wd - 1) // stride + 1
    if not store and not want_stat:
        raise ValueError("dwconv3x3(store=False) leaves nothing but the statistic: want_stat must be set")
    if x_codes_out is not None:
        if store:
            raise ValueError("dwconv3x3 keeps the codes of x only in its statistic pass (store=False)")
        _check_front_codes(x_codes_out, "x_codes_out", tuple(x.shape), x.device)
    y = torch.empty((n, c, ho, wo), dtype=torch.float32, device=x.device) if store else None
    stat, zflag = _stat_target(n, x.device, want_stat)
    check_call(_lib_().fq_dwconv3x3(_ptr(x), _ptr(w), _ptr(bias), _ptr(y), n, c, h, wd, int(stride), _ptr(in_stat),
                                    _ptr(in_thr), int(width), int(flags), _ptr(cur_out), _ptr(bn_scale),
                                    _ptr(bn_shift), _ACTS[act] | zflag, _ptr(stat), _stream(x), _ptr(x_codes_out)))
    return y, stat


def dwconv3x3_c16(x, w, bias=None, stride=1, in_stat=None, in_thr=None, width=8, flags=0, cur_out=None, bn_scale=None,
                  bn_shift=None, act=None, want_stat=True, out_codes=None):
    if not isinstance(x, Codes16) or in_thr is None or not x.matches(in_thr, width, flags):
        raise ValueError("dwconv3x3_c16 wants a Codes16 input quantised with this call's in_thr / width / signedness")
    if out_codes is None:
        raise ValueError("dwconv3x3_c16 writes codes: give out_codes")
    _check(x.t, "x", torch.int8)
    _check(w, "w")
    n, c, h, wd = x.shape
    if w.dim() != 4 or tuple(w.shape[1:]) != (1, 3, 3) or w.shape[0] != c:
        raise ValueError("dwconv3x3_c16 wants w (C,1,3,3); got %s for C = %d" % (tuple(w.shape), c))
    for name, t in (("bias", bias), ("in_stat", in_stat), ("in_thr", in_thr), ("bn_scale", bn_scale),
                    ("bn_shift", bn_shift), ("cur_out", cur_out)):
        if t is not None:
            _check(t, name)
    dev = x.t.device
    ho, wo = (h - 1) // stride + 1, (wd - 1) // stride + 1
    othr = _check(out_codes["thr"], "out_codes['thr']")
    y = Codes16.empty((n, c, ho, wo), dev, othr, out_codes.get("width", 8), out_codes.get("flags", 0))
    if in_stat is not None and cur_out is None:
        cur_out = torch.empty(1, dtype=torch.float32, device=dev)
    stat, zflag = _stat_target(n, dev, want_stat)
    check_call(_lib_().fq_dwconv3x3_c16(_ptr(x.t), _ptr(w), _ptr(bias), _ptr(y.t), n, c, h, wd, int(stride), _ptr(in_stat),
                                        _ptr(in_thr), int(width), int(flags), _ptr(cur_out), _ptr(bn_scale), _ptr(bn_shift),
                                        _ACTS[act] | zflag, _ptr(stat), _ptr(othr), y.width, y.flags, _stream(w)))
    return y, stat


def pwdw_supported(xshape, cout, stride):
    n, cin, h, w = (int(v) for v in xshape)
    lib = _lib_()
    return bool(lib.fq_pwconv_i8_stat_supported(n, cin, int(cout), h * w, 0, 0)) and \
        bool(lib.fq_pwdw_fused_supported(n, cin, int(cout), h, w, int(stride), 0))


def pwconv_front_supported(xshape, cout):
    n, cin, h, w = (int(v) for v in xshape)
    return bool(_lib_().fq_pwconv_i8_stat_supported(n, cin, int(cout), h * w, h, w))


def pair_codes_shape(xshape):
    n, cin, h, w = (int(v) for v in xshape)
    return (n, 2 * ((cin + 31) // 32), h * w, 16)


def _check_pair_codes(t, name, x):
    _check(t, name, torch.int8)
    if x.dim() != 4 or tuple(t.shape) != pair_codes_shape(x.shape):
        raise ValueError("%s must be int8 %s for x %s; got %s" % (name, pair_codes_shape(x.shape) if x.dim() == 4 else "(4-d x)",
                                                                  tuple(x.shape), tuple(t.shape)))
    if t.device != x.device:
        raise ValueError("%s lives on %s, x on %s" % (name, t.device, x.device))
    return t


def pwconv_i8_stat(x, wcodes, wscale, wsum, bias=None, in_stat=None, in_thr=None, width=8, flags=0, cur_out=None,
                   bn_scale=None, bn_shift=None, act=None, x_codes_out=None, front=None):
    _check(x, "x")
    _check(wcodes, "wcodes", torch.int8)
    _check(wscale, "wscale")
    _check(wsum, "wsum", torch.int32)
    for name, t in (("bias", bias), ("in_stat", in_stat), ("in_thr", in_thr), ("bn_scale", bn_scale),
                    ("bn_shift", bn_shift), ("cur_out", cur_out)):
        if t is not None:
            _check(t, name)
    n, cin = x.shape[0], x.shape[1]
    cout = wscale.numel()
    cin_pad = wcodes.shape[1]
    if (cin + 63) // 64 * 64 != cin_pad:
        raise ValueError("x has %d channels but the weight codes were made for a row length that pads to %d" % (cin, cin_pad))
    if in_stat is not None and cur_out is None:
        cur_out = torch.empty(1, dtype=torch.float32, device=x.device)
    if x_codes_out is not None:
        _check_pair_codes(x_codes_out, "x_codes_out", x)
    f_args = (_ptr(None),) * 5 + (0, _ptr(None), _ptr(None), 0, 0, 0, 0)
    if front is not None:
        unknown = set(front) - {"x_codes", "w", "bias", "bn_scale", "bn_shift", "act", "in_stat", "in_thr", "width", "flags"}
        if unknown or x.dim() != 4:
            raise ValueError("pwconv_i8_stat(front=) wants x (N, Cin, H, W) and the keys of a depthwise call; got %s, %s"
                             % (tuple(x.shape), sorted(unknown)))
        fw = _check(front["w"], "front['w']")
        if tuple(fw.shape) != (cin, 1, 3, 3):
            raise ValueError("front['w'] must be (%d,1,3,3); got %s" % (cin, tuple(fw.shape)))
        _check_front_codes(front["x_codes"], "front['x_codes']", tuple(x.shape), x.device)
        for name in ("bias", "bn_scale", "bn_shift", "in_stat", "in_thr"):
            if front.get(name) is not None:
                _check(front[name], "front['%s']" % name)
        if not pwconv_front_supported(x.shape, cout):
            raise ValueError("pwconv_i8_stat(front=) does not take x %s -> %d channels: see pwconv_front_supported"
                             % (tuple(x.shape), cout))
        f_args = (_ptr(front["x_codes"]), _ptr(fw), _ptr(front.get("bias")), _ptr(front.get("bn_scale")),
                  _ptr(front.get("bn_shift")), _ACTS[front.get("act")], _ptr(front.get("in_stat")), _ptr(front.get("in_thr")),
                  int(front.get("width", 8)), int(front.get("flags", 0)), int(x.shape[2]), int(x.shape[3]))
    stat, zflag = _stat_target(n, x.device, True)
    hw = x.numel() // (n * cin)
    check_call(_lib_().fq_pwconv_i8_stat(_ptr(x), _ptr(wcodes), _ptr(wscale), _ptr(wsum), _ptr(bias), n, cin, cin_pad,
                                         wcodes.shape[0], cout, hw, _ptr(in_stat), _ptr(in_thr), int(width), int(flags), _ptr(cur_out),
                                         _ptr(bn_scale), _ptr(bn_shift), _ACTS[act] | zflag, _ptr(stat), _ptr(x_codes_out),
                                         _stream(x), *f_args))
    return stat


def pwdw_chain_supported(xshape, cout):
    n, cin, h, w = (int(v) for v in xshape)
    lib = _lib_()
    return lib.fq_version() >= 102 and bool(lib.fq_pwdw_fused_supported(n, cin, int(cout), h, w, 1, 1))


def pwdw_fused(x, wcodes, wscale, wsum, dw_w, pw_bias=None, in_stat=None, in_thr=None, width=8, flags=0, pw_bn_scale=None,
               pw_bn_shift=None, pw_act=None, mid_stat=None, mid_thr=None, mid_width=8, mid_flags=0, mid_cur_out=None,
               dw_bias=None, stride=1, dw_bn_scale=None, dw_bn_shift=None, dw_act=None, want_stat=True, x_codes=None,
               store=True, mid_codes_out=None):
    _check(x, "x")
    _check(wcodes, "wcodes", torch.int8)
    _check(wscale, "wscale")
    _check(wsum, "wsum", torch.int32)
    _check(dw_w, "dw_w")
    for name, t in (("pw_bias", pw_bias), ("in_stat", in_stat), ("in_thr", in_thr), ("pw_bn_scale", pw_bn_scale),
                    ("pw_bn_shift", pw_bn_shift), ("mid_stat", mid_stat), ("mid_thr", mid_thr), ("mid_cur_out", mid_cur_out),
                    ("dw_bias", dw_bias), ("dw_bn_scale", dw_bn_scale), ("dw_bn_shift", dw_bn_shift)):
        if t is not None:
            _check(t, name)
    if x.dim() != 4:
        raise ValueError("pwdw_fused wants x (N, Cin, H, W); got %s" % (tuple(x.shape),))
    n, cin, h, w = x.shape
    cout = wscale.numel()
    if dw_w.dim() != 4 or tuple(dw_w.shape) != (cout, 1, 3, 3):
        raise ValueError("pwdw_fused wants dw_w (%d,1,3,3); got %s" % (cout, tuple(dw_w.shape)))
    cout_pad, cin_pad = wcodes.shape
    if (cin + 63) // 64 * 64 != cin_pad:
        raise ValueError("x has %d channels but the weight codes were made for a row length that pads to %d" % (cin, cin_pad))
    if x_codes is not None:
        _check_pair_codes(x_codes, "x_codes", x)
    ho, wo = (h - 1) // stride + 1, (w - 1) // stride + 1
    if (mid_codes_out is None) == (not store):
        raise ValueError("pwdw_fused keeps the codes of the 1x1 output in its statistic mode only: store=False and mid_codes_out "
                         "go together")
    if not store:
        if not want_stat or stride != 1 or x_codes is None:
            raise ValueError("pwdw_fused(store=False) wants want_stat, stride 1 and x_codes")
        _check_front_codes(mid_codes_out, "mid_codes_out", (n, cout, h, w), x.device)
        if not pwdw_chain_supported(x.shape, cout):
            raise ValueError("pwdw_fused(store=False) does not take x %s -> %d channels: see pwdw_chain_supported"
                             % (tuple(x.shape), cout))
    y = torch.empty((n, cout, ho, wo), dtype=torch.float32, device=x.device) if store else None
    stat, zflag = _stat_target(n, x.device, want_stat)
    check_call(_lib_().fq_pwdw_fused(_ptr(x), _ptr(wcodes), _ptr(wscale), _ptr(wsum), _ptr(pw_bias), n, cin, cin_pad, cout_pad,
                                     cout, h, w, _ptr(in_stat), _ptr(in_thr), int(width), int(flags), _ptr(pw_bn_scale),
                                     _ptr(pw_bn_shift), _ACTS[pw_act], _ptr(mid_stat), _ptr(mid_thr), int(mid_width),
                                     int(mid_flags), _ptr(mid_cur_out), _ptr(dw_w), _ptr(dw_bias), int(stride),
                                     _ptr(dw_bn_scale), _ptr(dw_bn_shift), _ACTS[dw_act] | zflag, _ptr(y), _ptr(stat),
                                     _ptr(x_codes), _stream(x), _ptr(mid_codes_out)))
    return y, stat


def weight_codes(w, rows_per_scale, width=8):
    _check(w, "w")
    rows = w.shape[0]
    row_len = w.numel() // rows
    row_pad = (row_len + 63) // 64 * 64
    rows_pad = (rows + 63) // 64 * 64
    buf = torch.empty(2 * rows_pad * row_pad, dtype=torch.int8, device=w.device)
    codes = buf[:rows_pad * row_pad].view(rows_pad, row_pad)
    scales = torch.empty(rows, dtype=torch.float32, device=w.device)
    rowsum = torch.empty(rows, dtype=torch.int32, device=w.device)
    ws = _workspace(w.device, _lib_().fq_weight_workspace_bytes(rows))
    check_call(_lib_().fq_weight_codes(_ptr(w), rows, row_len, int(rows_per_scale), int(width), row_pad, rows_pad,
                                       _ptr(codes), _ptr(scales), _ptr(rowsum), _ptr(ws), _stream(w)))
    return codes, scales, rowsum


def weight_codes_reproduce(w, codes, scales):
    rows = w.shape[0]
    w2 = w.reshape(rows, -1)
    back = codes[:rows, :w2.shape[1]].to(torch.float32) * scales.reshape(rows, 1)
    return bool(torch.equal(back, w2))


class Codes16(object):
    __slots__ = ("t", "shape", "thr", "width", "flags")

    def __init__(self, t, shape, thr, width, flags):
        self.t, self.shape, self.thr, self.width, self.flags = t, tuple(int(d) for d in shape), thr, int(width), int(flags)

    @staticmethod
    def empty(shape, device, thr, width, flags):
        n, c, h, w = shape
        t = torch.empty((n, (c + 15) // 16, h * w, 16), dtype=torch.int8, device=device)
        return Codes16(t, shape, thr, width, flags)

    def matches(self, thr, width, flags):
        return self.thr.data_ptr() == thr.data_ptr() and self.width == int(width) and \
            (self.flags & 3) == (int(flags) & 3)


PW_FORMS = {None: 0, "auto": 0, "two_kernels": 1, "stream": 3, "split": 6, "sample": 7, "rows": 8}


SPLIT_KT = (2, 4, 6, 8, 10, 12, 16, 18, 30, 32, 64)


def pwconv_strided_supported(cin):
    return ((int(cin) + 63) // 64 * 64) // 32 in SPLIT_KT


def pwconv_residual_supported(cin):
    return ((int(cin) + 63) // 64 * 64) // 32 in SPLIT_KT


def pwconv_shortcut_supported(cin, cin2, cout):
    return bool(_lib_().fq_pwconv_i8_shortcut_supported(int(cin), int(cin2), int(cout)))


def pwconv_i8_shortcut(x, wcodes, wscale, wsum, bias=None, in_stat=None, in_thr=None, width=8, flags=0, cur_out=None,
                       bn_scale=None, bn_shift=None, act=None, x2=None, wcodes2=None, wscale2=None, wsum2=None, in_stat2=None,
                       in_thr2=None, width2=8, flags2=0, cur_out2=None, bn_scale2=None, bn_shift2=None, side_codes=None):
    a16, b16 = isinstance(x, Codes16), isinstance(x2, Codes16)
    if a16 != (side_codes is not None) or (b16 and not a16):
        raise ValueError("pwconv_i8_shortcut: fp32 on every side, or a Codes16 x with side_codes (x2 then fp32 or Codes16)")
    if a16 and (in_thr is None or not x.matches(in_thr, width, flags)):
        raise ValueError("the C16 input was quantised with another threshold / width / signedness than this call names")
    if b16 and (in_thr2 is None or not x2.matches(in_thr2, width2, flags2)):
        raise ValueError("the C16 shortcut input was quantised with another threshold / width / signedness than this call names")
    xt, x2t = (x.t if a16 else x), (x2.t if b16 else x2)
    xs, x2s = (x.shape if a16 else tuple(x.shape)), (x2.shape if b16 else tuple(x2.shape))
    for name, t, dt in (("x", xt, torch.int8 if a16 else None), ("wcodes", wcodes, torch.int8), ("wscale", wscale, None),
                        ("wsum", wsum, torch.int32), ("x2", x2t, torch.int8 if b16 else None), ("wcodes2", wcodes2, torch.int8),
                        ("wscale2", wscale2, None), ("wsum2", wsum2, torch.int32), ("bn_scale2", bn_scale2, None),
                        ("bn_shift2", bn_shift2, None)):
        if dt is None:
            _check(t, name)
        else:
            _check(t, name, dt)
    for name, t in (("bias", bias), ("in_stat", in_stat), ("in_thr", in_thr), ("bn_scale", bn_scale), ("bn_shift", bn_shift),
                    ("cur_out", cur_out), ("in_stat2", in_stat2), ("in_thr2", in_thr2), ("cur_out2", cur_out2)):
        if t is not None:
            _check(t, name)
    if len(xs) != 4 or len(x2s) != 4 or tuple(xs[2:]) != tuple(x2s[2:]) or xs[0] != x2s[0]:
        raise ValueError("pwconv_i8_shortcut wants x (N, Cin, H, W) and x2 (N, Cin2, H, W); got %s and %s" % (tuple(xs), tuple(x2s)))
    n, cin, h, w = xs
    cin2 = x2s[1]
    dev = xt.device
    cout = wscale.numel()
    if wscale2.numel() != cout:
        raise ValueError("the two convolutions must have the same number of filters (%d and %d)" % (cout, wscale2.numel()))
    if wcodes.shape[1] != cin or wcodes2.shape[1] != cin2 or not pwconv_shortcut_supported(cin, cin2, cout):
        raise ValueError("pwconv_i8_shortcut: %d / %d -> %d channels is not a shape it takes" % (cin, cin2, cout))
    if in_stat is not None and cur_out is None:
        cur_out = torch.empty(1, dtype=torch.float32, device=dev)
    if in_stat2 is not None and cur_out2 is None:
        cur_out2 = torch.empty(1, dtype=torch.float32, device=dev)
    y = torch.empty((n, cout, h, w), dtype=torch.float32, device=dev)
    stat, zflag = _stat_target(n, dev, True)
    if not a16:
        check_call(_lib_().fq_pwconv_i8_shortcut(_ptr(xt), _ptr(wcodes), _ptr(wscale), _ptr(wsum), _ptr(bias), _ptr(y), n, cin, cin,
                                                 cout, h * w, _ptr(in_stat), _ptr(in_thr), int(width), int(flags), _ptr(cur_out),
                                                 _ptr(bn_scale), _ptr(bn_shift), _ACTS[act] | zflag, _ptr(stat), _ptr(x2t),
                                                 _ptr(wcodes2), _ptr(wscale2), _ptr(wsum2), cin2, cin2, _ptr(in_stat2), _ptr(in_thr2),
                                                 int(width2), int(flags2), _ptr(cur_out2), _ptr(bn_scale2), _ptr(bn_shift2),
                                                 _stream(xt)))
        return y, stat
    sthr = _check(side_codes["thr"], "side_codes['thr']")
    y16 = Codes16.empty((n, cout, h, w), dev, sthr, side_codes.get("width", 8), side_codes.get("flags", 0))
    check_call(_lib_().fq_pwconv_i8_shortcut_c16(_ptr(xt), _ptr(wcodes), _ptr(wscale), _ptr(wsum), _ptr(bias), _ptr(y), _ptr(y16.t), n,
                                                 cin, cin, cout, h * w, _ptr(in_stat), _ptr(in_thr), int(width), int(flags),
                                                 _ptr(cur_out), _ptr(bn_scale), _ptr(bn_shift), _ACTS[act] | zflag, _ptr(stat),
                                                 _ptr(x2t), 1 if b16 else 0, _ptr(wcodes2), _ptr(wscale2), _ptr(wsum2), cin2, cin2,
                                                 _ptr(in_stat2), _ptr(in_thr2), int(width2), int(flags2), _ptr(cur_out2),
                                                 _ptr(bn_scale2), _ptr(bn_shift2), _ptr(sthr), int(y16.width), int(y16.flags),
                                                 _stream(wcodes)))
    return y, stat, y16


def pwconv_gap_supported(xshape, cout, residual=False):
    if len(xshape) != 4:
        return False
    return bool(_lib_().fq_pwconv_i8_gap_supported(int(xshape[0]), int(xshape[1]), int(cout), int(xshape[2]) * int(xshape[3]),
                                                    1 if residual else 0))


def pwconv_i8_gap(x, wcodes, wscale, wsum, bias=None, in_stat=None, in_thr=None, width=8, flags=0, cur_out=None,
                  bn_scale=None, bn_shift=None, act=None, residual=None):
    _check(x, "x")
    _check(wcodes, "wcodes", torch.int8)
    _check(wscale, "wscale")
    _check(wsum, "wsum", torch.int32)
    for name, t in (("bias", bias), ("in_stat", in_stat), ("in_thr", in_thr), ("bn_scale", bn_scale), ("bn_shift", bn_shift),
                    ("cur_out", cur_out), ("residual", residual)):
        if t is not None:
            _check(t, name)
    if x.dim() != 4:
        raise ValueError("pwconv_i8_gap wants x (N, Cin, H, W); got %s" % (tuple(x.shape),))
    n, cin, h, w = x.shape
    cout = wscale.numel()
    cin_pad = wcodes.shape[1]
    if cin != cin_pad:
        raise ValueError("pwconv_i8_gap: Cin = %d must be a multiple of 64" % cin)
    if residual is not None and tuple(residual.shape) != (n, cout, h, w):
        raise ValueError("the residual must have the convolution output's shape %s, got %s" % ((n, cout, h, w), tuple(residual.shape)))
    if not pwconv_gap_supported(tuple(x.shape), cout, residual is not None):
        raise ValueError("pwconv_i8_gap: shape %s -> %d channels is not taken (fq_pwconv_i8_gap_supported)" % (tuple(x.shape), cout))
    if in_stat is not None and cur_out is None:
        cur_out = torch.empty(1, dtype=torch.float32, device=x.device)
    y = torch.empty((n, cout, 1, 1), dtype=torch.float32, device=x.device)
    stat, zflag = _stat_target(n, x.device, True)
    ws = torch.empty(_lib_().fq_pwconv_workspace_bytes(n, cin_pad, h * w), dtype=torch.uint8, device=x.device)
    check_call(_lib_().fq_pwconv_i8_gap(_ptr(x), _ptr(wcodes), _ptr(wscale), _ptr(wsum), _ptr(bias), _ptr(y), n, cin, cin_pad, cout,
                                        h * w, _ptr(in_stat), _ptr(in_thr), int(width), int(flags), _ptr(cur_out), _ptr(bn_scale),
                                        _ptr(bn_shift), _ACTS[act] | zflag, _ptr(stat), _ptr(residual), _ptr(ws), _stream(x)))
    return y, stat


def pwconv_sub2_supported(cin, cout):
    return bool(_lib_().fq_pwconv_i8_sub2_supported(int(cin), int(cout)))


def pwconv_i8(x, wcodes, wscale, wsum, bias=None, in_stat=None, in_thr=None, width=8, flags=0, cur_out=None,
              bn_scale=None, bn_shift=None, act=None, want_stat=True, form=None, stride=1, residual=None, out_codes=None,
              side_codes=None, subsample=False):
    in16 = isinstance(x, Codes16)
    if subsample:
        if (in16 and side_codes is None) or out_codes is not None or stride != 1 or len(x.shape) != 4:
            raise ValueError("subsample=True goes with (N, Cin, H, W) activations, stride 1 and fp32 output (codes in: with "
                             "side_codes, fq_pwconv_i8_c16_dual_sub2)")
        if not pwconv_sub2_supported(x.shape[1], wscale.numel()):
            raise ValueError("subsample=True: %d -> %d channels is not a shape fq_pwconv_i8_sub2 takes" % (x.shape[1], wscale.numel()))
    if in16:
        if in_thr is None or not x.matches(in_thr, width, flags):
            raise ValueError("the C16 input was quantised with another threshold / width / signedness than this call names")
        xs = x.shape
        _check(x.t, "x", torch.int8)
    else:
        _check(x, "x")
        xs = tuple(x.shape)
    _check(wcodes, "wcodes", torch.int8)
    _check(wscale, "wscale")
    _check(wsum, "wsum", torch.int32)
    for name, t in (("bias", bias), ("in_stat", in_stat), ("in_thr", in_thr), ("bn_scale", bn_scale),
                    ("bn_shift", bn_shift), ("cur_out", cur_out), ("residual", residual)):
        if t is not None:
            _check(t, name)
    n, cin = xs[0], xs[1]
    dev = x.t.device if in16 else x.device
    cout = wscale.numel()
    cin_pad = wcodes.shape[1]
    if (cin + 63) // 64 * 64 != cin_pad:
        raise ValueError("x has %d channels but the weight codes were made for a row length that pads to %d"
                         % (cin, cin_pad))
    if in_stat is not None and cur_out is None:
        cur_out = torch.empty(1, dtype=torch.float32, device=dev)
    stat, zflag = _stat_target(n, dev, want_stat)
    if side_codes is not None:
        if not in16 or residual is None or stride != 1 or out_codes is not None or len(xs) != 4:
            raise ValueError("side_codes goes with a Codes16 input, a residual operand, stride 1 and fp32 output")
        h, w = xs[2], xs[3]
        hs, ws_ = ((h + 1) // 2, (w + 1) // 2) if subsample else (h, w)
        y = torch.empty((n, cout, hs, ws_), dtype=torch.float32, device=dev)
        if tuple(residual.shape) != (n, cout, h, w):
            raise ValueError("the residual must have the whole output's shape %s, got %s" % ((n, cout, h, w), tuple(residual.shape)))
        sthr = _check(side_codes["thr"], "side_codes['thr']")
        y16 = Codes16.empty((n, cout, hs, ws_), dev, sthr, side_codes.get("width", 8), side_codes.get("flags", 0))
        ws = torch.empty(_lib_().fq_pwconv_workspace_bytes(n, cin_pad, h * w), dtype=torch.uint8, device=dev)
        check_call((_lib_().fq_pwconv_i8_c16_dual_sub2 if subsample else _lib_().fq_pwconv_i8_c16_dual)(_ptr(x.t), _ptr(wcodes), _ptr(wscale), _ptr(wsum), _ptr(bias), _ptr(y),
                                                 _ptr(y16.t), n, cin, cin_pad, cout, h, w, _ptr(in_stat), _ptr(in_thr),
                                                 int(width), int(flags), _ptr(cur_out), _ptr(bn_scale), _ptr(bn_shift),
                                                 _ACTS[act] | zflag, _ptr(stat), _ptr(residual), _ptr(sthr), int(y16.width),
                                                 int(y16.flags), _ptr(ws), _stream(wcodes)))
        return y, stat, y16
    if in16 or out_codes is not None:
        if len(xs) != 4:
            raise ValueError("a C16 hand-over needs (N, Cin, H, W) activations, got %s" % (xs,))
        h, w = xs[2], xs[3]
        ho, wo = (h - 1) // stride + 1, (w - 1) // stride + 1
        if out_codes is not None:
            if residual is not None:
                raise ValueError("a residual operand goes with fp32 output")
            othr = _check(out_codes["thr"], "out_codes['thr']")
            y = Codes16.empty((n, cout, ho, wo), dev, othr, out_codes.get("width", 8), out_codes.get("flags", 0))
            yp, ow, of = _ptr(y.t), y.width, y.flags
        else:
            y = torch.empty((n, cout, ho, wo), dtype=torch.float32, device=dev)
            if residual is not None and tuple(residual.shape) != tuple(y.shape):
                raise ValueError("the residual must have the output's shape %s, got %s" % (tuple(y.shape), tuple(residual.shape)))
            othr, yp, ow, of = None, _ptr(y), 8, 0
        ws = torch.empty(_lib_().fq_pwconv_workspace_bytes(n, cin_pad, ho * wo), dtype=torch.uint8, device=dev)
        check_call(_lib_().fq_pwconv_i8_c16(_ptr(x.t if in16 else x), 1 if in16 else 0, _ptr(wcodes), _ptr(wscale), _ptr(wsum),
                                            _ptr(bias), yp, n, cin, cin_pad, cout, h, w, int(stride), _ptr(in_stat),
                                            _ptr(in_thr), int(width), int(flags), _ptr(cur_out), _ptr(bn_scale),
                                            _ptr(bn_shift), _ACTS[act] | zflag, _ptr(stat), _ptr(residual), _ptr(othr),
                                            int(ow), int(of), _ptr(ws), _stream(wcodes)))
        return y, stat
    if subsample:
        h, w = x.shape[2], x.shape[3]
        y = torch.empty((n, cout, (h + 1) // 2, (w + 1) // 2), dtype=torch.float32, device=x.device)
        if residual is not None and tuple(residual.shape) != (n, cout, h, w):
            raise ValueError("the residual must have the whole output's shape %s, got %s" % ((n, cout, h, w), tuple(residual.shape)))
        ws = torch.empty(_lib_().fq_pwconv_workspace_bytes(n, cin_pad, h * w), dtype=torch.uint8, device=x.device)
        check_call(_lib_().fq_pwconv_i8_sub2(_ptr(x), _ptr(wcodes), _ptr(wscale), _ptr(wsum), _ptr(bias), _ptr(y), n, cin, cin_pad,
                                             cout, h, w, _ptr(in_stat), _ptr(in_thr), int(width), int(flags), _ptr(cur_out),
                                             _ptr(bn_scale), _ptr(bn_shift), _ACTS[act] | zflag, _ptr(stat), _ptr(residual),
                                             _ptr(ws), _stream(x)))
        return y, stat
    if stride != 1 or residual is not None:
        if x.dim() != 4:
            raise ValueError("a strided 1x1 convolution needs (N, Cin, H, W) activations, got %s" % (tuple(x.shape),))
        h, w = x.shape[2], x.shape[3]
        ho, wo = (h - 1) // stride + 1, (w - 1) // stride + 1
        y = torch.empty((n, cout, ho, wo), dtype=torch.float32, device=x.device)
        if residual is not None and tuple(residual.shape) != tuple(y.shape):
# ... 378 lines not shown
```

quantization/mxnet_amd/quantize/convert/convert_conv2d.py:

```python
from collections import namedtuple

import os

import torch

from ...mx import nd
from ...mx import autograd
from ...mx.ndarray import NDArray
from ...mx.gluon.nn import Conv2D
from ... import ops
from .._state import DeviceScalar
from ._blocks import INPUT_RANGE, BatchNormTerms, contiguous, rebind_forward, scalar_slot

__all__ = ['gen_conv2d_converter']

QuantizedArgs = namedtuple("ConvQuantizedArgs",
                           "quantize_input in_signed in_width "
                           "wt_width quant_type "
                           "fake_bn wino_quantize")

WINOGRAD_VARIANTS = ("F23", "F43", "F63")


def current_slot(block, like):
# ... 32 lines not shown


def fake_quant_block_input(block, x, input_max, flags, width):
    v = _InputView(block, x)
    wanted = block.quantize_input
    offline = block.quantize_input_offline
    y = None
    if v.exchange is not None and v.rows is not None:
        v.exchange(v.per_sample(), v.n, v.cur)
        if wanted:
            y = ops.fake_quant_offline(v.t, input_max._t if offline else v.cur, width, flags, want_stat=False)[0]
    elif v.hint is not None or (v.rows is not None and getattr(block, "_fq_keep_rows", False)):
        stat = v.per_sample()
        if wanted and not offline:
            y = ops.fake_quant_online_prestat(v.t, stat, width, flags, cur_out=v.cur)[0]
        else:
            ops.batch_mean(stat, out=v.cur)
            if wanted:
                y = ops.fake_quant_offline(v.t, input_max._t, width, flags, want_stat=False)[0]
    elif not wanted:
        ops.batch_mean(v.per_sample(), out=v.cur)
    elif offline:
        y = ops.fake_quant_offline(v.t, input_max._t, width, flags, cur_out=v.cur, stat_ws=v.rows,
                                   want_stat=getattr(block, "track_input_stat", True))[0]
    else:
        y = ops.fake_quant_online(v.t, width, flags, cur_out=v.cur, stat_ws=v.rows)[0]
    v.finish(block)
    if y is None:
        return x
    return NDArray(autograd.ste_link(v.t, y))


def fused_input_plan(block, x, input_max, flags, width):
    v = _InputView(block, x)
    wanted = block.quantize_input
    online = wanted and not block.quantize_input_offline
    stat = None
    if online or v.exchange is not None or getattr(block, "track_input_stat", True):
        stat = v.per_sample()
    plan = {}
    if v.exchange is not None and v.rows is not None:
        v.exchange(stat, v.n, v.cur)
        if wanted:
            plan = dict(in_thr=input_max._t if block.quantize_input_offline else v.cur, width=width, flags=flags)
    elif online:
        plan = dict(in_stat=stat, width=width, flags=flags, cur_out=v.cur)
    elif wanted:
        plan = dict(in_thr=input_max._t, width=width, flags=flags)
        if stat is not None:
            plan.update(in_stat=stat, cur_out=v.cur)
    elif stat is not None:
        ops.batch_mean(stat, out=v.cur)
    v.finish(block)
    return plan


def depthwise_fused(block, x, weight_q, bias, plan):
    fz = block._fq_dw_fused
    scale, shift = fz["constants"]() if fz["bn"] is not None else (None, None)
    c16_in = getattr(x, "_fq_c16", None)
    if c16_in is not None:
        out_codes = handover_target(block, fz) if "in_thr" in plan else None
        if out_codes is not None:
            yc, stat = ops.dwconv3x3_c16(c16_in, contiguous(weight_q._t), None if bias is None else bias._t,
                                         stride=block._kwargs["stride"][0], bn_scale=scale, bn_shift=shift, act=fz["act"],
                                         out_codes=out_codes, **plan)
            out = NDArray(yc.t)
            out._fq_c16 = yc
            out._fq_stat = stat
            return out
        x = NDArray(codes16_to_fake_quant(c16_in))
        plan = {}
    call = dict(x=contiguous(x._t), w=contiguous(weight_q._t), bias=None if bias is None else bias._t,
                stride=block._kwargs["stride"][0], bn_scale=scale, bn_shift=shift, act=fz["act"], **plan)
    front = front_target(block, fz, x, plan) if c16_in is None else None
    if front is not None:
        xcodes = torch.empty(ops.front_codes_shape(call["x"].shape), dtype=torch.int8, device=call["x"].device)
        stat = _dwconv3x3(call, store=False, x_codes_out=xcodes)[1]
        out = NDArray(_placeholder(tuple(call["x"].shape), call["x"].device))
        out._fq_stat = stat
        out._fq_deferred = dict(kind="front", consumer=front, call=call, x_codes=xcodes)
        return out
    y, stat = _dwconv3x3(call)
    out = NDArray(y)
    out._fq_stat = stat
    return out


def _dwconv3x3(call, **more):
    kw = dict(call)
    return ops.dwconv3x3(kw.pop("x"), **kw, **more)


def front_target(block, fz, x, plan, level=None):
    from .. import fuse as _fuse
    nxt = fz.get("front_pw")
    level = int(_fuse.PAIR_FRONT) if level is None else int(level)
    if nxt is None or not _fuse.PAIR_CODES or not (level >= 2 or (level and ops.in_flight())) \
            or block._kwargs["stride"] != (1, 1) \
            or block.quantize_args.fake_bn or "in_stat" not in plan or "in_thr" in plan or plan["width"] > 8:
        return None
    pz, a = nxt._fq_pw_fused, nxt.quantize_args
    if not (nxt.enable_quantize and a.quantize_input and nxt.quantize_input and not nxt.quantize_input_offline
            and a.in_width <= 8 and a.wt_width <= 8 and not getattr(nxt, "_fq_no_int8", False) and not a.fake_bn
            and getattr(nxt, "_fq_global_stat", None) is None and getattr(nxt, "_fq_residual", None) is None):
        return None
    if any(_hooked(b) for b in (block, fz.get("bn"), fz.get("act_block"))):
        return None
    if recompute_target(nxt, pz, x, dict(in_stat=None), None) is None or handover_target(nxt) is not None:
        return None
    if not ops.pwconv_front_supported(tuple(x._t.shape), nxt._kwargs["num_filter"]):
        return None
    return nxt


def _weight_rows_per_scale(block, args):
    cout = block._kwargs["num_filter"]
    per_channel = args.quant_type == "channel" or (args.quant_type == "group" and block._kwargs["num_group"] == cout)
    return 1 if per_channel else cout


def _pointwise_weight_codes(block, args, weight_raw, weight_q):
    param_t = block.weight.data()._t
    key = (param_t.data_ptr(), param_t._version)
    held = getattr(block, "_fq_pw_cache", None)
    if block.fixed_params == 1 and held is not None and held[3] == key:
        return held[:3]
    three = block._fq_pw_fused.get("kind") == "3x3"
    if block._fq_pw_fused.get("sliced"):
        codes = ops.weight_slices_3x3(contiguous(weight_q._t))
        if block.fixed_params == 1:
            block._fq_pw_cache = tuple(codes) + (key,)
        return codes
    make = ops.weight_codes_3x3 if three else ops.weight_codes
    rederived = block.fixed_params == 1 and held is not None
    src = contiguous((weight_q if rederived else weight_raw)._t)
    live = None if rederived else block.__dict__.get("_fq_pw_live")
    if live is not None and live[0] is weight_raw._t and live[1] == weight_raw._t._version:
        codes = live[2]
    else:
        codes = make(src, _weight_rows_per_scale(block, args), args.wt_width)
        if not rederived and block.fixed_params != 1 and weight_raw._t is param_t:
            block.__dict__["_fq_pw_live"] = (weight_raw._t, weight_raw._t._version, codes)
    if block.fixed_params == 1:
        block.__dict__.pop("_fq_pw_live", None)
    if rederived:
        ref = src.permute(0, 2, 3, 1).contiguous() if three else src
        if not ops.weight_codes_reproduce(ref, codes[0], codes[1]):
            block._fq_no_int8 = True
            block.__dict__.pop("_fq_pw_cache", None)
            return None
    if block.fixed_params == 1:
        block._fq_pw_cache = tuple(codes) + (key,)
    return codes


_DW_C16_MIN_PIXELS = int(os.environ.get("FQ_DW_C16_MIN_PIXELS", "1"))


def _consumer_takes_codes(nxt):
    a = nxt.quantize_args
    return (nxt.enable_quantize and a.quantize_input and nxt.quantize_input and nxt.quantize_input_offline
            and a.in_width <= 8 and a.wt_width <= 8 and not getattr(nxt, "_fq_no_int8", False)
            and getattr(nxt, "input_max", None) is not None and getattr(nxt, "_fq_global_stat", None) is None)


def _hooked(b):
    return b is not None and bool(getattr(b, "_forward_hooks", None) or getattr(b, "_forward_pre_hooks", None))


def handover_target(block, fz=None):
    from .. import fuse as _fuse
    fz = fz if fz is not None else block._fq_pw_fused
    nxt = fz.get("next")
    if nxt is None or not _fuse.HANDOVER or autograd.is_recording() or not _consumer_takes_codes(nxt):
        return None
    if any(_hooked(b) for b in (block, nxt, fz.get("bn"), fz.get("act_block")) + tuple(fz.get("via", ()))):
        return None
    dw = getattr(nxt, "_fq_dw_fused", None)
    if dw is not None and (handover_target(nxt, dw) is None or not fz.get("c16_pays", True)):
        return None
    a = nxt.quantize_args
    return dict(thr=nxt.input_max.data()._t, width=a.in_width, flags=ops.act_flags(signed=a.in_signed))


def _same_quantiser(block, other, plan, codes):
    from .. import fuse as _fuse
    if not _fuse.SIDE_CODES or codes.width != int(plan["width"]) or (codes.flags & 3) != (int(plan["flags"]) & 3):
        return False
    ta, tb = plan["in_thr"], getattr(other, "input_max", None)
    if tb is None:
        return False
    tb = tb.data()._t
    if tb.data_ptr() != codes.thr.data_ptr():
        return False
    key = (ta.data_ptr(), ta._version, tb.data_ptr(), tb._version, ops.state_epoch())
    memo = block.__dict__.get("_fq_same_thr")
    if memo is None or memo[0] != key:
        if ta.is_cuda and torch.cuda.is_current_stream_capturing():
            return False
        memo = block.__dict__["_fq_same_thr"] = (key, bool(torch.equal(ta.reshape(-1)[:1], tb.reshape(-1)[:1])))
    return memo[1]


_THIN_FORMS = os.environ.get("FQ_PWS_THIN", "1") != "0"
_SIDE_MAX_CIN = int(os.environ.get("FQ_SIDE_MAX_CIN", "512"))


def side_target(block, c16_in):
    from .. import fuse as _fuse
    nxt = block._fq_pw_fused.get("side_next")
    if nxt is None or c16_in is None or not _fuse.SIDE_CODES or not _fuse.HANDOVER or autograd.is_recording():
        return None
    if not _consumer_takes_codes(nxt) or getattr(nxt, "_fq_pw_fused", None) is None or nxt.quantize_args.in_signed:
        return None
    cin, cout = c16_in.shape[1], block._kwargs["num_filter"]
    if cin not in (64, 128, 256, 512) or cin > _SIDE_MAX_CIN or cout % 32 or cout < 256:
        return None
    return nxt


def sub_target(block, fz, xshape):
    from .. import fuse as _fuse
    link = fz.get("sub_next")
    if link is None or not _fuse.SUBSAMPLE or autograd.is_recording() or _fuse._collection is not None:
        return None
    if getattr(ops.StatArena._tls, "current", None) is None or len(xshape) != 4:
        return None
    for r in link["readers"]:
        k = r._kwargs
        if k["kernel"] != (1, 1) or k["stride"] != (2, 2) or k["pad"] != (0, 0) or getattr(r, "_fq_pw_fused", None) is None:
            return None
    if any(_hooked(b) for b in (block, fz.get("bn"), fz.get("act_block")) + tuple(link["readers"]) + tuple(link["via"])):
        return None
    for r in link["readers"]:
        rz = r._fq_pw_fused
        if any(_hooked(b) for b in (rz.get("bn"), rz.get("act_block"))):
            return None
    if not ops.pwconv_sub2_supported(xshape[1], block._kwargs["num_filter"]):
        return None
    return link


def gap_target(block, fz, c16_in, xshape, residual):
    from .. import fuse as _fuse
    link = fz.get("gap_next")
    if link is None or not _fuse.GAP_FUSE or c16_in is not None or autograd.is_recording() or _fuse._collection is not None:
        return None
    if getattr(ops.StatArena._tls, "current", None) is None or block._kwargs["stride"] != (1, 1):
        return None
    if any(_hooked(b) for b in (block, fz.get("bn"), fz.get("act_block"), link["gap"]) + tuple(link["via"])):
        return None
    if not ops.pwconv_gap_supported(xshape, block._kwargs["num_filter"], residual):
        return None
    return link["gap"]


def defer_shortcut(block, fz, x, x_arg, c16_in, codes3, bias, scale, shift, plan, stride_, extra):
    from .. import fuse as _fuse
    if not getattr(block, "_fq_defer_short", False):
        return None
    block._fq_defer_short = False
    if extra or bias is not None or scale is None or fz["act"] != "none" or stride_ != 1:
        return None
    if c16_in is not None and "in_thr" not in plan:
        return None
    if autograd.is_recording() or _fuse._collection is not None or getattr(ops.StatArena._tls, "current", None) is None:
        return None
    if any(_hooked(b) for b in (block, fz.get("bn"))) or not plan:
        return None
    xs = tuple(x_arg.shape)
    dev = x_arg.t.device if isinstance(x_arg, ops.Codes16) else x_arg.device
    out = NDArray(_placeholder((xs[0], block._kwargs["num_filter"], xs[2], xs[3]), dev))
    out._fq_short = dict(x=x_arg, codes=codes3, bn=(scale, shift), plan=dict(plan), block=block)
    return out


def materialise_shortcut_record(d):
    return ops.pwconv_i8(d["x"], *d["codes"], None, bn_scale=d["bn"][0], bn_shift=d["bn"][1], act=None, want_stat=False,
                         **d["plan"])[0]


def materialise_shortcut(s):
    return NDArray(materialise_shortcut_record(s._fq_short))


def _convolve(block, F, x, weight, bias):
    if getattr(x, "_fq_sub2", None) is None:
        return block.origin_forward(F, x, weight, bias)
    out = F.Convolution(x, weight, bias, name="fwd", **dict(block._kwargs, stride=(1, 1)))
    return out if block.act is None else block.act(out)


_PLACEHOLDERS = {}


def _placeholder(shape, device):
    one = _PLACEHOLDERS.get(device)
    if one is None:
        one = _PLACEHOLDERS[device] = torch.zeros(1, dtype=torch.int8, device=device)
    return one.expand(*shape)


def recompute_target(block, fz, x, plan, c16_in):
    from .. import fuse as _fuse
    nxt = fz.get("pair_dw")
    if nxt is None or not _fuse.RECOMPUTE or c16_in is not None or autograd.is_recording() or _fuse._collection is not None:
        return None
    if getattr(ops.StatArena._tls, "current", None) is None:
        return None
    if "in_stat" not in plan or "in_thr" in plan or getattr(block, "_fq_residual", None) is not None:
        return None
    a = nxt.quantize_args
    if not (nxt.enable_quantize and a.quantize_input and nxt.quantize_input and not nxt.quantize_input_offline
            and getattr(nxt, "_fq_global_stat", None) is None and not a.fake_bn and nxt._kwargs["num_group"] == block._kwargs["num_filter"]):
        return None
    if any(_hooked(b) for b in (block, nxt, fz.get("bn"), fz.get("act_block"))):
        return None
    t = x._t
    if t.dim() != 4 or t.shape[2] * t.shape[3] < _fuse.RECOMPUTE_MIN_PIXELS or t.shape[1] > _fuse.RECOMPUTE_MAX_CIN:
        return None
    if not ops.pwdw_supported(tuple(t.shape), block._kwargs["num_filter"], nxt._kwargs["stride"][0]):
        return None
    return nxt


def _front_tensor(front):
    return front["store"]() if front.get("store") is not None else _dwconv3x3(front["call"])


def _materialise(x):
    d = x._fq_deferred
    if d.get("kind") == "front":
        y, stat = _front_tensor(d)
    else:
        src = d["x"] if d.get("front") is None else _front_tensor(d["front"])[0]
        y, stat = ops.pwconv_i8(src, *d["codes"], d["bias"], bn_scale=d["bn"][0], bn_shift=d["bn"][1], act=d["act"],
                                **d["plan"])
    out = NDArray(y)
    out._fq_stat = stat
    return out


def chain_target(block, fz, x, d, width):
    from .. import fuse as _fuse
    if d.get("x_codes") is None or fz.get("front_pw") is None:
        return None
    nxt = front_target(block, fz, x, dict(in_stat=x._fq_stat, width=width), level=_fuse.PAIR_CHAIN)
    if nxt is None or not ops.pwdw_chain_supported(tuple(d["x"].shape), block._kwargs["num_filter"]):
        return None
    return nxt


def depthwise_recompute(block, x, weight_q, bias, flags, width):
    d = x._fq_deferred
    fz = block._fq_dw_fused
    scale, shift = fz["constants"]() if fz["bn"] is not None else (None, None)
    src = d["x"]
    n = src.shape[0]
    cur, side = scalar_slot(block, src)
    stat = x._fq_stat
    rows = getattr(block, "_fq_stat_ws", None)
    if rows is not None and rows.device == src.device and rows.numel() >= n:
        rows[:n].copy_(stat)
    p = d["plan"]
    dw_w, dw_b = contiguous(weight_q._t), None if bias is None else bias._t

    def fused(**more):
        return ops.pwdw_fused(src, *d["codes"], dw_w, pw_bias=d["bias"], in_stat=p["in_stat"],
                              width=p["width"], flags=p["flags"], pw_bn_scale=d["bn"][0], pw_bn_shift=d["bn"][1],
                              pw_act=d["act"], mid_stat=stat, mid_width=width, mid_flags=flags, mid_cur_out=cur,
                              dw_bias=dw_b, stride=block._kwargs["stride"][0],
                              dw_bn_scale=scale, dw_bn_shift=shift, dw_act=fz["act"], x_codes=d.get("x_codes"), **more)
    chain = chain_target(block, fz, x, d, width)
    if chain is not None:
        oshape = tuple(x._t.shape)
        ycodes = torch.empty(ops.front_codes_shape(oshape), dtype=torch.int8, device=src.device)
        zstat = fused(store=False, mid_codes_out=ycodes)[1]
        out = NDArray(_placeholder(oshape, src.device))
        out._fq_stat = zstat
        out._fq_deferred = dict(kind="front", consumer=chain, x_codes=ycodes, store=fused,
                                call=dict(w=dw_w, bias=dw_b, bn_scale=scale, bn_shift=shift, act=fz["act"], in_stat=stat,
                                          width=width, flags=flags))
    else:
        z, zstat = fused()
        out = NDArray(z)
        out._fq_stat = zstat
    if not side:
        block._fq_last_n = n
        block.current_input_max = DeviceScalar(cur)
    return out


def _handed_over(x):
    return getattr(x, "_fq_c16", None)


def codes16_to_fake_quant(c16):
    n, c, h, w = c16.shape
    signed = bool(c16.flags & 1)
    b = (c16.t.to(torch.int16) & 255) ^ 0x80
    codes = (b - 128).to(torch.int8).to(torch.float32) if signed else b.to(torch.float32)
    levels = float((1 << (c16.width - 1)) - 1) if signed else float((1 << c16.width) - 1)
    scale = c16.thr.reshape(()) / levels
    t = codes.reshape(n, -1, h * w, 16).permute(0, 1, 3, 2).reshape(n, -1, h, w)[:, :c]
    return (t * scale).contiguous()


def pointwise_fused(block, F, x, weight_raw, weight_q, bias, plan, weights_quantised):
    fz = block._fq_pw_fused
    args = block.quantize_args
    scale, shift = fz["constants"]() if fz["bn"] is not None else (None, None)
    on_codes = bool(plan) and weights_quantised and args.in_width <= 8 and args.wt_width <= 8 \
        and not getattr(block, "_fq_no_int8", False)
    held = _pointwise_weight_codes(block, args, weight_raw, weight_q) if on_codes else None
    on_codes = held is not None
    front = getattr(x, "_fq_deferred", None)
    if front is not None:
        from .. import fuse as _fuse
        if not (on_codes and fz.get("kind") == "1x1" and _fuse.PAIR_CODES and getattr(block, "_fq_residual", None) is None
                and handover_target(block) is None and recompute_target(block, fz, x, plan, None) is not None):
            x, front = _materialise(x), None
    res0 = getattr(block, "_fq_residual", None)
    if res0 is not None and res0.get("short") is not None and not (on_codes and fz.get("kind") == "1x1"):
        res0["t"], res0["short"] = materialise_shortcut_record(res0["short"]), None
    c16_in = _handed_over(x)
    stride_ = 1 if getattr(x, "_fq_sub2", None) is not None else block._kwargs["stride"][0]
    if c16_in is None and on_codes and "in_thr" in plan:
        side = getattr(x, "_fq_side", None)
        if side is not None and not autograd.is_recording():
            if side[0] is block and side[1].matches(plan["in_thr"], plan["width"], plan["flags"]):
                c16_in = side[1]
            elif side[0] is not block and _same_quantiser(block, side[0], plan, side[1]):
                c16_in = ops.Codes16(side[1].t, side[1].shape, plan["in_thr"], plan["width"], plan["flags"])
    if c16_in is not None and not (on_codes and "in_thr" in plan):
        x = NDArray(codes16_to_fake_quant(c16_in))
        plan, c16_in = {}, None
    if on_codes:
        codes, scales, rowsum = held
        if front is not None:
            x_arg = torch.empty(tuple(x._t.shape), dtype=torch.float32, device=x._t.device)
        else:
            x_arg = c16_in if c16_in is not None else contiguous(x._t)
        if fz.get("kind") == "3x3":
            out_codes = None if fz.get("sliced") else handover_target(block)
            y, stat = ops.conv3x3_i8(x_arg, codes, scales, rowsum, None if bias is None else bias._t,
                                     bn_scale=scale, bn_shift=shift, act=fz["act"],
                                     **({} if fz.get("sliced") or out_codes is None else dict(out_codes=out_codes)), **plan)
        else:
            res = getattr(block, "_fq_residual", None)
            extra = {}
            xshape = c16_in.shape if c16_in is not None else tuple(x._t.shape)
            side_blk = sub_link = None
            if res is not None and res.get("short") is not None:
                d = res["short"]
                side_s = side_target(block, c16_in) if c16_in is not None else None
                d16 = isinstance(d["x"], ops.Codes16)
                if (block._kwargs["stride"][0] == 1 and scale is not None and not _hooked(block)
                        and (c16_in is None and not d16 or (side_s is not None and "in_thr" in plan))
                        and tuple(d["x"].shape[2:]) == tuple(xshape[2:]) and d["x"].shape[0] == xshape[0]
                        and ops.pwconv_shortcut_supported(xshape[1], d["x"].shape[1], block._kwargs["num_filter"])
                        and (c16_in is None or block._kwargs["num_filter"] % 512 == 0 or xshape[1] == 64)
                        and not autograd.is_recording()):
                    p2 = d["plan"]
                    kw2 = dict(x2=d["x"], wcodes2=d["codes"][0], wscale2=d["codes"][1], wsum2=d["codes"][2], in_stat2=p2.get("in_stat"),
                               in_thr2=p2.get("in_thr"), width2=p2["width"], flags2=p2["flags"], cur_out2=p2.get("cur_out"),
                               bn_scale2=d["bn"][0], bn_shift2=d["bn"][1])
                    if side_s is not None:
                        a_ = side_s.quantize_args
                        kw2["side_codes"] = dict(thr=side_s.input_max.data()._t, width=a_.in_width, flags=ops.act_flags(signed=a_.in_signed))
                    out = ops.pwconv_i8_shortcut(x_arg, codes, scales, rowsum, None if bias is None else bias._t, bn_scale=scale,
                                                 bn_shift=shift, act=res["act"], **kw2, **plan)
                    res["used"] = True
                    folded = NDArray(out[0])
                    folded._fq_stat = out[1]
                    if side_s is not None:
                        folded._fq_side = (side_s, out[2])
                    return folded
                res["t"] = materialise_shortcut_record(d)
                res["short"] = None
            if res is not None and block._kwargs["stride"][0] == 1 and tuple(res["t"].shape[2:]) == tuple(xshape[2:]) \
                    and res["t"].shape[1] == block._kwargs["num_filter"] and ops.pwconv_residual_supported(xshape[1]):
                extra = dict(residual=res["t"])
                res["used"] = True
                side_blk = side_target(block, c16_in)
                if side_blk is not None:
                    a_ = side_blk.quantize_args
                    extra["side_codes"] = dict(thr=side_blk.input_max.data()._t, width=a_.in_width,
                                               flags=ops.act_flags(signed=a_.in_signed))
                if side_blk is not None or c16_in is None:
                    sub_link = sub_target(block, fz, xshape)
                    if sub_link is not None:
                        extra["subsample"] = True
            if not extra and (c16_in is None or xshape[1] >= 256 or
                              (xshape[1] <= 32 and xshape[0] * xshape[2] * xshape[3] > 32 * 4096 and _THIN_FORMS)):
                xs = c16_in.shape if c16_in is not None else tuple(x._t.shape)
                s_ = stride_
                fz["c16_pays"] = len(xs) == 4 and ((xs[2] - 1) // s_ + 1) * ((xs[3] - 1) // s_ + 1) >= _DW_C16_MIN_PIXELS
                out_codes = handover_target(block)
                if out_codes is not None and fz.get("via") is not None:
                    co = block._kwargs["num_filter"]
                    if not (co >= 256 or (co <= 32 and xs[0] * ((xs[2] - 1) // s_ + 1) * ((xs[3] - 1) // s_ + 1) > 32 * 4096
                                          and _THIN_FORMS)):
                        out_codes = None
                if out_codes is not None:
                    extra = dict(out_codes=out_codes)
            if not extra or (set(extra) == {"residual"} and side_blk is None):
                gap = gap_target(block, fz, c16_in, xshape, "residual" in extra)
                if gap is not None:
                    y, stat = ops.pwconv_i8_gap(x_arg, codes, scales, rowsum, None if bias is None else bias._t, bn_scale=scale,
                                                bn_shift=shift, act=res["act"] if "residual" in extra else fz["act"],
                                                residual=extra.get("residual"), **plan)
                    pooled = NDArray(y)
                    pooled._fq_stat = stat
                    pooled._fq_pooled_by = gap
                    return pooled
            short = defer_shortcut(block, fz, x, x_arg, c16_in, (codes, scales, rowsum), bias, scale, shift, plan, stride_, extra)
            if short is not None:
                return short
            pair = recompute_target(block, fz, x, plan, c16_in) if not extra else None
            if pair is not None:
                b_ = None if bias is None else bias._t
                from .. import fuse as _fuse
                xcodes = torch.empty(ops.pair_codes_shape(x_arg.shape), dtype=torch.int8, device=x_arg.device) \
                    if _fuse.PAIR_CODES else None
                fkw = {}
                if front is not None:
                    c_ = front["call"]
                    fkw = dict(front=dict(x_codes=front["x_codes"], w=c_["w"], bias=c_["bias"], bn_scale=c_["bn_scale"],
                                          bn_shift=c_["bn_shift"], act=c_["act"], in_stat=c_["in_stat"], width=c_["width"],
                                          flags=c_["flags"]))
                stat = ops.pwconv_i8_stat(x_arg, codes, scales, rowsum, b_, bn_scale=scale, bn_shift=shift, act=fz["act"],
                                          x_codes_out=xcodes, **fkw, **plan)
                xs = tuple(x_arg.shape)
                res_ = NDArray(_placeholder((xs[0], block._kwargs["num_filter"], xs[2], xs[3]), x_arg.device))
                res_._fq_stat = stat
                res_._fq_deferred = dict(x=x_arg, codes=(codes, scales, rowsum), bias=b_, bn=(scale, shift), act=fz["act"],
                                         plan=dict(in_stat=plan["in_stat"], width=plan["width"], flags=plan["flags"],
                                                   cur_out=plan.get("cur_out")), consumer=pair, x_codes=xcodes, front=front)
                return res_
            out = ops.pwconv_i8(x_arg, codes, scales, rowsum, None if bias is None else bias._t,
                                bn_scale=scale, bn_shift=shift,
                                act=res["act"] if "residual" in extra else fz["act"],
                                stride=stride_, **extra, **plan)
            y, stat = out[0], out[1]
            if sub_link is not None and side_blk is None:
                trunk = NDArray(y)
                trunk._fq_stat = stat
                trunk._fq_sub2 = {"hw": tuple(xshape[2:]), "readers": sub_link["readers"], "unit": sub_link["unit"]}
                return trunk
            if side_blk is not None:
                trunk = NDArray(y)
                trunk._fq_stat = stat
                trunk._fq_side = (side_blk, out[2])
                if sub_link is not None:
                    trunk._fq_sub2 = {"hw": tuple(xshape[2:]), "readers": sub_link["readers"], "unit": sub_link["unit"]}
                return trunk
    else:
        if plan:
            t = contiguous(x._t)
            if "in_thr" not in plan:
                xq = ops.fake_quant_online_prestat(t, plan["in_stat"], plan["width"], plan["flags"],
                                                   cur_out=plan.get("cur_out"))[0]
            else:
                if "in_stat" in plan:
                    ops.batch_mean(plan["in_stat"], out=plan["cur_out"])
                xq = ops.fake_quant_offline(t, plan["in_thr"], plan["width"], plan["flags"], want_stat=False)[0]
            xq_ = NDArray(xq)
            xq_._fq_sub2 = x._fq_sub2
            x = xq_
        out = _convolve(block, F, x, weight_q, bias)
        from .. import fuse as _fuse
        res = getattr(block, "_fq_residual", None)
        if (res is not None and scale is not None and fz["act"] == "none" and res.get("owner") is not None and _fuse.BN_ADD
                and tuple(res["t"].shape) == tuple(out._t.shape) and out._t.is_cuda):
            owner = res["owner"]
            sink = _fuse._kl_sink(owner)
            y, stat = ops.bn_act_stat(contiguous(out._t), scale, shift, res["act"], hist=sink, residual=res["t"])
            res["used"] = True
            r_ = NDArray(y)
            r_._fq_stat = stat
            if _fuse._collection is not None:
                r_._fq_kl = (owner, sink)
            return r_
        if fz["bn"] is None and fz["act"] == "none":
            return out
        if scale is None:
            c = out.shape[1]
            scale = torch.ones(c, dtype=torch.float32, device=out._t.device)
            shift = torch.zeros(c, dtype=torch.float32, device=out._t.device)
        sink = _fuse._kl_sink(block)
        y, stat = ops.bn_act_stat(out._t.contiguous(), scale, shift, fz["act"], hist=sink)
        res = NDArray(y)
        res._fq_stat = stat
        if _fuse._collection is not None:
            res._fq_kl = (block, sink)
        return res
    if isinstance(y, ops.Codes16):
        res = NDArray(y.t)
        res._fq_c16 = y
    else:
        res = NDArray(y)
    res._fq_stat = stat
    return res


def _fake_quant_weight(block, args, weight):
    keep = not args.fake_bn and not autograd.is_recording()
    if keep:
        held = block.__dict__.get("_fq_wq_cache")
        if held is not None and held[0] is weight._t and held[1] == weight._t._version:
            return held[2]
    out = _fake_quant_weight_now(block, args, weight)
    if keep:
        block.__dict__["_fq_wq_cache"] = (weight._t, weight._t._version, out)
    return out


def _fake_quant_weight_now(block, args, weight):
    w = contiguous(weight._t)
    if args.quant_type == 'channel' and args.wino_quantize != 'none' and block._kwargs['kernel'] == (3, 3):
        wq = ops.wino_weight_fake_quant(w, args.wino_quantize, args.wt_width)
        return NDArray(autograd.wino_link(w, wq, *ops.winograd_matrices(args.wino_quantize)))
    if args.quant_type == 'channel':
        rows = block._kwargs['num_filter']
    elif args.quant_type == 'group':
        rows = block._kwargs['num_group']
        if rows not in (1, w.shape[0]):
            raise ValueError("group-wise weight quantisation needs num_group in {1, num_filter} "
                             "(got num_group=%d, num_filter=%d): operands could not be broadcast" % (rows, w.shape[0]))
    else:
        rows = 1
    return NDArray(autograd.ste_link(w, ops.weight_fake_quant(w, rows, args.wt_width)))


def _quantised_conv(self, F, x, weight, bias=None, input_max=None,
                    gamma=None, beta=None, running_mean=None, running_var=None):
    args = self.quantize_args
    dw = getattr(self, "_fq_dw_fused", None)
    pw = getattr(self, "_fq_pw_fused", None)
    taken_over = dw is not None or pw is not None
    if taken_over and autograd.is_recording():
        raise RuntimeError("this net was rewired by quantize.fuse.fuse_inference (inference only): call "
                           "quantize.fuse.unfuse(net) before recording gradients")
    frozen = self.fixed_params == 1
    weight_raw, plan = weight, {}

    if args.fake_bn and not frozen:
        terms = BatchNormTerms(gamma, beta, running_mean, running_var)
        weight, bias = terms.fold_weight(F, weight), terms.fold_bias(F, bias)

# ... 89 lines not shown
```

quantization/mxnet_amd/quantize/fuse.py:

```python
import types

import torch

from ..mx.gluon import nn
from ..mx.ndarray import NDArray
from .. import ops

__all__ = ["fuse_inference", "unfuse", "refresh", "eval_head", "EvalHead"]


def _is_relu6_block(b):
    return type(b).__name__ == "RELU6"


def _act_kind(b):
    if isinstance(b, nn.Activation) and b._act_type == "relu" and not hasattr(b, "quantize_args") \
            and b.hybrid_forward.__func__ is nn.Activation.hybrid_forward:
        return "relu"
    if _is_relu6_block(b):
        return "relu6"
    return None


def _tensors_key(*tensors):
    return tuple((t.data_ptr(), t._version) for t in tensors)


def _bn_constants(bn):
    g0, b = bn.gamma.data()._t, bn.beta.data()._t
    mean, var = bn.running_mean.data()._t, bn.running_var.data()._t
    g = torch.ones_like(g0) if bn._kwargs.get("fix_gamma", False) else g0
    scale = g / torch.sqrt(var + bn._kwargs["eps"])
    shift = b - mean * scale
    return scale.contiguous(), shift.contiguous(), _tensors_key(g0, b, mean, var)


_collection = None
_collection_calls = {}


def begin_collection():
    global _collection
    _collection = {}
    _collection_calls.clear()
    return _collection


def end_collection():
    global _collection
    _collection = None
    _collection_calls.clear()


def collection_calls():
    return _collection_calls


def _kl_sink(producer):
    if _collection is None:
        return None
    _collection_calls[producer] = _collection_calls.get(producer, 0) + 1
    return _collection.get(producer)


def _fused_bn_forward(self, F, x, gamma, beta, running_mean, running_var):
    st = self._fq_fused
    key = _tensors_key(gamma._t, beta._t, running_mean._t, running_var._t)
    if st["key"] != key:
        st["scale"], st["shift"], st["key"] = _bn_constants(self)
    t = x._t if x._t.is_contiguous() else x._t.contiguous()
    if st.get("pool") is not None and t.dim() == 4 and t.shape[3] % 4 == 0:
        y, stat = ops.bn_act_maxpool_stat(t, st["scale"], st["shift"], st["act"], want_stat=True)
        out = NDArray(y)
        out._fq_stat = stat
        out._fq_pooled_by = st["pool"]
        return out
    else:
        sink = _kl_sink(self)
        y, stat = ops.bn_act_stat(t, st["scale"], st["shift"], st["act"], want_stat=True, hist=sink)
        out = NDArray(y)
        out._fq_stat = stat
        if _collection is not None:
            out._fq_kl = (self, sink)
        return out


def _pool_after_bn_forward(self, F, x):
    if getattr(x, "_fq_pooled_by", None) is self:
        x._fq_pooled_by = None
        return x
    return self._fq_pool_fused["orig"](F, x)


def _pool_stat_forward(self, F, x):
    if getattr(x, "_fq_pooled_by", None) is self:
        x._fq_pooled_by = None
        return x
    t = x._t if x._t.is_contiguous() else x._t.contiguous()
    if t.dim() != 4 or t.shape[3] % 4 or not t.is_cuda:
        return self._fq_pool_fused["orig"](F, x)
    st = self._fq_pool_fused
    c = t.shape[1]
    if st.get("ones") is None or st["ones"].numel() != c or st["ones"].device != t.device:
        st["ones"] = torch.ones(c, dtype=torch.float32, device=t.device)
        st["zeros"] = torch.zeros(c, dtype=torch.float32, device=t.device)
    y, stat = ops.bn_act_maxpool_stat(t, st["ones"], st["zeros"], "none", want_stat=True)
    out = NDArray(y)
    out._fq_stat = stat
    return out


def _is_maxpool_3x3s2p1(b):
    if type(b) is not nn.MaxPool2D or b.hybrid_forward.__func__ is not nn.MaxPool2D.hybrid_forward:
        return False
    k = b._kwargs
    return (k["kernel"] == (3, 3) and k["stride"] == (2, 2) and k["pad"] == (1, 1) and not k["global_pool"]
            and k["pooling_convention"] == "valid")


import os as _os

HANDOVER = _os.environ.get("FQ_HANDOVER", "1") != "0"
SIDE_CODES = _os.environ.get("FQ_HANDOVER_SIDE", "1") != "0"
STEM_CODES = _os.environ.get("FQ_HANDOVER_STEM", "1") != "0"
WINO_SLICED = _os.environ.get("FQ_WINO_SLICED", "1") != "0"
BN_ADD = _os.environ.get("FQ_BN_ADD", "1") != "0"
RECOMPUTE = _os.environ.get("FQ_RECOMPUTE", "1") != "0"
RECOMPUTE_MIN_PIXELS = int(_os.environ.get("FQ_RECOMPUTE_MIN_PIXELS", "3136"))
RECOMPUTE_MAX_CIN = int(_os.environ.get("FQ_RECOMPUTE_MAX_CIN", "128"))
PAIR_CODES = _os.environ.get("FQ_PWDW_CODES", "1") != "0"
PAIR_FRONT = int(_os.environ.get("FQ_PWDW_FRONT", "1"))
PAIR_CHAIN = int(_os.environ.get("FQ_PWDW_CHAIN", "1"))
SUBSAMPLE = _os.environ.get("FQ_SUBSAMPLE", "1") != "0"
GAP_FUSE = _os.environ.get("FQ_GAP_FUSE", "1") != "0"
SHORTCUT_FUSE = _os.environ.get("FQ_SHORTCUT_FUSE", "1") != "0"
UNIT_LINKS = _os.environ.get("FQ_HANDOVER_UNITS", "1") != "0"


def _identity_forward(self, F, x, *args, **kwargs):
    return x


def _is_dw3x3(b):
    if type(b) is not nn.Conv2D:
        return False
    k = b._kwargs
    cin = b.weight.shape[1] if b.weight.shape else 0
    return (k["kernel"] == (3, 3) and k["pad"] == (1, 1) and k["dilate"] == (1, 1) and k["stride"] in ((1, 1), (2, 2))
            and k["num_group"] == k["num_filter"] and cin == 1 and k["layout"] == "NCHW" and b.act is None
            and not getattr(getattr(b, "quantize_args", None), "fake_bn", False))


def _is_pw1x1(b):
    if type(b) is not nn.Conv2D or not hasattr(b, "quantize_args"):
        return False
    k = b._kwargs
    if not (k["kernel"] == (1, 1) and k["pad"] == (0, 0) and k["dilate"] == (1, 1) and k["num_group"] == 1
            and k["layout"] == "NCHW" and b.act is None and not b.quantize_args.fake_bn):
        return False
    if k["stride"] == (1, 1):
        return True
    cin = b.weight.shape[1] if b.weight.shape is not None and len(b.weight.shape) == 4 else 0
    return k["stride"] == (2, 2) and cin > 0 and ops.pwconv_strided_supported(cin)


def _is_dense3x3(b):
    if type(b) is not nn.Conv2D or not hasattr(b, "quantize_args"):
        return False
    k = b._kwargs
    a = b.quantize_args
    cin = b.weight.shape[1] if b.weight.shape is not None and len(b.weight.shape) == 4 else 0
    return (k["kernel"] == (3, 3) and k["pad"] == (1, 1) and k["dilate"] == (1, 1) and k["stride"] == (1, 1)
            and k["num_group"] == 1 and k["layout"] == "NCHW" and b.act is None and not a.fake_bn
            and cin in (64, 128, 256, 512) and k["num_filter"] >= 32
            and (not _wino_sliced(b) or (k["num_filter"] % 32 == 0 and WINO_SLICED)))


def _wino_sliced(b):
    a = b.quantize_args
    return a.quant_type == "channel" and a.wino_quantize != "none"


def _is_stem3x3s2(b):
    if type(b) is not nn.Conv2D or hasattr(b, "quantize_args"):
        return False
    if b.hybrid_forward.__func__ is not nn.Conv2D.hybrid_forward:
        return False
    k = b._kwargs
    shp = b.weight.shape
    return (len(shp) == 4 and k["num_group"] == 1 and k["dilate"] == (1, 1) and k["layout"] == "NCHW" and b.act is None
            and ops.stem_conv_supported(shp[1], shp[0], k["kernel"], k["stride"], k["pad"]))


def _stem_forward(self, F, x, weight, bias=None):
    st = self._fq_stem_fused
    w = weight._t
    key = (w.data_ptr(), w._version)
    if st["wkey"] != key:
        st["wt"], st["wkey"] = w.permute(1, 2, 3, 0).contiguous(), key
    scale = shift = None
    if st["constants"] is not None:
        scale, shift = st["constants"]()
    t = x._t if x._t.is_contiguous() else x._t.contiguous()
    out_codes = None
    if st.get("next") is not None and w.shape[2] == 3 and STEM_CODES:
        from .convert.convert_conv2d import handover_target
        out_codes = handover_target(self, st)
    pool = st.get("pool")
    hooked = any(bool(getattr(b, "_forward_hooks", None) or getattr(b, "_forward_pre_hooks", None))
                 for b in (self, st.get("bn"), st.get("act_block"), pool) if b is not None)
    pooled = (pool is not None and STEM_POOL and out_codes is None and w.shape[2] == 7 and t.dim() == 4 and not hooked
              and ops.stem_pool_supported(t.shape[2], t.shape[3]))
    y, stat = ops.stem_conv_s2(t, w, None if bias is None else bias._t, bn_scale=scale, bn_shift=shift,
                               act=st["act"], want_stat=True, w_tap_major=st["wt"], pool=pooled,
                               **({} if out_codes is None else dict(out_codes=out_codes)))
    if out_codes is not None:
        out = NDArray(y.t)
        out._fq_c16 = y
    else:
        out = NDArray(y)
    if pooled:
        out._fq_pooled_by = pool
    out._fq_stat = stat
    return out


def _gap_stat_forward(self, F, x):
    if getattr(x, "_fq_pooled_by", None) is self:
        x._fq_pooled_by = None
        return x
    t = x._t if x._t.is_contiguous() else x._t.contiguous()
    y, stat = ops.global_avg_pool_stat(t, want_stat=True)
    out = NDArray(y)
    out._fq_stat = stat
    return out


def _flatten_keep_stat_forward(self, F, x):
    out = NDArray(x._t.reshape(x._t.shape[0], -1))
    out._fq_stat = x._fq_stat
    return out


def _plain_dw_forward(self, F, x, weight, bias=None):
    from .convert.convert_conv2d import depthwise_fused
    return depthwise_fused(self, x, weight, bias, {})


def _tail_conv(seq):
    kids = list(seq._children.values()) if isinstance(seq, (nn.Sequential, nn.HybridSequential)) else []
    if kids and isinstance(kids[-1], (nn.Sequential, nn.HybridSequential)):
        return _tail_conv(kids[-1])
    if len(kids) < 2 or type(kids[-1]) is not nn.BatchNorm:
        return None
    conv, bn = kids[-2], kids[-1]
    fz = getattr(conv, "_fq_pw_fused", None)
    if fz is None or fz.get("kind") != "1x1" or fz["bn"] is not bn or fz["act"] != "none":
        return None
    return conv if conv._kwargs["stride"] == (1, 1) else None


def _with_residual(conv, shortcut, act, run, owner=None):
    short = getattr(shortcut, "_fq_short", None)
    t = None if short is not None else (shortcut._t if shortcut._t.is_contiguous() else shortcut._t.contiguous())
    conv._fq_residual = {"t": t, "short": short, "act": act, "used": False, "owner": owner}
    try:
        out = run()
        return out, conv._fq_residual["used"]
    finally:
        conv._fq_residual = None


def _residual_unit_forward(self, x):
    from ..mx import autograd
    if autograd.is_recording():
        raise RuntimeError("this net was rewired by quantize.fuse.fuse_inference (inference only): call "
                           "quantize.fuse.unfuse(net) before recording gradients")
    sub = getattr(x, "_fq_sub2", None)
    if sub is not None and sub["unit"] is not self:
        raise RuntimeError("a subsampled trunk (fq_pwconv_i8_sub2) reached a unit it was not made for")
    tail = _tail_conv(self.body)
    sc = _shortcut_conv(self) if (tail is not None and SHORTCUT_FUSE) else None
    if sc is not None:
        sc._fq_defer_short = True
    try:
        shortcut = x if self.downsample is None else self.downsample(x)
    finally:
        if sc is not None:
            sc._fq_defer_short = False
    if tail is not None:
        h, consumed = _with_residual(tail, shortcut, "relu", lambda: self.body(x), owner=self)
        if consumed:
            return h
    else:
        h = self.body(x)
    if getattr(shortcut, "_fq_short", None) is not None:
        from .convert.convert_conv2d import materialise_shortcut
        shortcut = materialise_shortcut(shortcut)
    a = h._t if h._t.is_contiguous() else h._t.contiguous()
    b = shortcut._t if shortcut._t.is_contiguous() else shortcut._t.contiguous()
    sink = _kl_sink(self)
    y, stat = ops.add_act_stat(a, b, "relu", want_stat=True, hist=sink)
    out = NDArray(y)
    out._fq_stat = stat
    if _collection is not None:
        out._fq_kl = (self, sink)
    return out


def _shortcut_conv(unit):
    ds = getattr(unit, "downsample", None)
    if type(ds) not in (nn.Sequential, nn.HybridSequential) or "forward" in ds.__dict__:
        return None
    kids = list(ds._children.values())
    if len(kids) != 2 or type(kids[0]) is not nn.Conv2D or type(kids[1]) is not nn.BatchNorm:
        return None
    fz = getattr(kids[0], "_fq_pw_fused", None)
    if fz is None or fz.get("kind") != "1x1" or fz["bn"] is not kids[1] or fz["act"] != "none":
        return None
    return kids[0]


def _linear_bottleneck_forward(self, x):
    from ..mx import autograd
    if autograd.is_recording():
        raise RuntimeError("this net was rewired by quantize.fuse.fuse_inference (inference only): call "
                           "quantize.fuse.unfuse(net) before recording gradients")
    tail = _tail_conv(self.out) if self.use_shortcut else None
    if tail is None:
        out = self.out(x)
        return out + x if self.use_shortcut else out
    out, consumed = _with_residual(tail, x, "none", lambda: self.out(x))
    return out if consumed else out + x


def _is_linear_bottleneck(b):
    from ..mx.gluon import model_zoo as zoo
    return getattr(type(b), "forward", None) is zoo.LinearBottleneck.forward and hasattr(b, "out") \
        and "forward" not in b.__dict__


def _is_residual_unit(b):
    from ..mx.gluon import model_zoo as zoo
    fwd = getattr(type(b), "forward", None)
    return fwd in (zoo.BasicBlockV1.forward, zoo.BottleneckV1.forward) and hasattr(b, "body") \
        and "forward" not in b.__dict__


def _bn_constants_getter(bn):
    cache = {"key": None, "val": None}

    def get():
        key = _tensors_key(bn.gamma.data()._t, bn.beta.data()._t, bn.running_mean.data()._t,
                           bn.running_var.data()._t) + (bn.__dict__.get("_fq_refresh", 0),)
        if cache["key"] != key:
            scale, shift, _ = _bn_constants(bn)
            cache["key"], cache["val"] = key, (scale, shift)
        return cache["val"]
    return get


def fuse_inference(net, depthwise=True, pointwise_int8=True, stem=True, residual=True, dense_int8=None):
    from .convert.convert import bump_mode_epoch
    bump_mode_epoch()
    if dense_int8 is None:
        dense_int8 = DENSE_INT8
    fused = [0]

    def bypass(blk):
        blk._fq_bypassed_orig = blk.hybrid_forward
        blk.hybrid_forward = types.MethodType(_identity_forward, blk)

    def visit_dw(container):
        if not isinstance(container, (nn.Sequential, nn.HybridSequential)):
            return
        kids = list(container._children.values())
        for i, b in enumerate(kids):
            if not _is_dw3x3(b) or hasattr(b, "_fq_dw_fused"):
                continue
            converted = hasattr(b, "quantize_args")
            if not converted and b.hybrid_forward.__func__ is not nn.Conv2D.hybrid_forward:
                continue
            bn = kids[i + 1] if i + 1 < len(kids) else None
            if not (type(bn) is nn.BatchNorm and not hasattr(bn, "_fq_fused") and bn._kwargs.get("axis", 1) == 1
                    and bn.hybrid_forward.__func__ is nn.BatchNorm.hybrid_forward):
                bn = None
            nxt = kids[i + 2] if bn is not None and i + 2 < len(kids) else (kids[i + 1] if bn is None and i + 1 < len(kids) else None)
            act = _act_kind(nxt) if nxt is not None else None
            b._fq_dw_fused = {"bn": bn, "act": act or "none", "act_block": nxt if act else None,
                              "constants": _bn_constants_getter(bn) if bn is not None else None,
                              "orig": None if converted else b.hybrid_forward}
            if not converted:
                b.hybrid_forward = types.MethodType(_plain_dw_forward, b)
            if bn is not None:
                bn._fq_fused = {"taken_by_conv": True, "orig": bn.hybrid_forward, "act_block": None}
                bn.hybrid_forward = types.MethodType(_identity_forward, bn)
            if act:
                bypass(nxt)
            fused[0] += 1

    def visit_stem(container):
        if not isinstance(container, (nn.Sequential, nn.HybridSequential)):
            return
        kids = list(container._children.values())
        for i, b in enumerate(kids):
            if not _is_stem3x3s2(b) or hasattr(b, "_fq_stem_fused"):
                continue
            bn = kids[i + 1] if i + 1 < len(kids) else None
            if not (type(bn) is nn.BatchNorm and not hasattr(bn, "_fq_fused") and bn._kwargs.get("axis", 1) == 1
                    and bn.hybrid_forward.__func__ is nn.BatchNorm.hybrid_forward):
                bn = None
            nxt = kids[i + 2] if bn is not None and i + 2 < len(kids) else (kids[i + 1] if bn is None and i + 1 < len(kids) else None)
            act = _act_kind(nxt) if nxt is not None else None
            b._fq_stem_fused = {"bn": bn, "act": act or "none", "act_block": nxt if act else None, "wt": None, "wkey": None,
                                "constants": _bn_constants_getter(bn) if bn is not None else None,
                                "orig": b.hybrid_forward}
            b.hybrid_forward = types.MethodType(_stem_forward, b)
            if bn is not None:
                bn._fq_fused = {"taken_by_conv": True, "orig": bn.hybrid_forward, "act_block": None}
                bn.hybrid_forward = types.MethodType(_identity_forward, bn)
            if act:
                bypass(nxt)
            j = i + 1 + (1 if bn is not None else 0) + (1 if act else 0)
            pool = kids[j] if j < len(kids) and _is_maxpool_3x3s2p1(kids[j]) and not hasattr(kids[j], "_fq_pool_fused") \
                else None
            if pool is not None:
                pool._fq_pool_fused = {"orig": pool.hybrid_forward}
                pool.hybrid_forward = types.MethodType(_pool_stat_forward, pool)
                b._fq_stem_fused["pool"] = pool
            b._fq_stem_fused["stem_follower"] = (container, j) if pool is None else None
            fused[0] += 1

    def link_stem(b):
        st = getattr(b, "_fq_stem_fused", None)
        if st is None or st.get("stem_follower") is None:
# ... 361 lines not shown
```

Baseline: 164,000.

## Extend pw-dw pair fusion to tail layers with an eight-wave 256-channel front kernel

Adds an eight-wavefront variant of the pointwise stat kernel that handles a 256-channel depthwise front layer, sharing one min/max table and splitting output-channel tiles across waves, with a larger LDS budget and one workgroup per CU. Python gating lets later, smaller-spatial layers take the pw-dw recompute/chain path behind a new FQ_PWDW_TAIL level (default off). The chain path for those shapes now uses the tail level, and the pair planner computes occupancy from held LDS when no output is stored. This trades lower occupancy and larger LDS for fewer intermediate tensor round trips in the network tail.

```diff
diff --git a/quantization/mxnet_amd/csrc/fq_core.hip b/quantization/mxnet_amd/csrc/fq_core.hip
--- a/quantization/mxnet_amd/csrc/fq_core.hip
+++ b/quantization/mxnet_amd/csrc/fq_core.hip
@@ -79,7 +79,7 @@
 extern "C" {
 
 const char* fq_last_error(void) { return g_err; }
-int fq_version(void) { return 102; }
+int fq_version(void) { return 103; }
 #ifndef FQ_BUILD_ID
 #define FQ_BUILD_ID "0000000000000000000000000000000000000000"
 #endif
diff --git a/quantization/mxnet_amd/csrc/fq_front_layout.h b/quantization/mxnet_amd/csrc/fq_front_layout.h
--- a/quantization/mxnet_amd/csrc/fq_front_layout.h
+++ b/quantization/mxnet_amd/csrc/fq_front_layout.h
@@ -14,6 +14,7 @@
 constexpr int kFrontRows = 8;
 constexpr int kFrontBandBytes = 32768;
 constexpr int kStatLdsPerCU = 160 * 1024, kStatLdsMax = 120 * 1024;
+constexpr int kStatLdsMaxWide = 150 * 1024;
 
 struct FrontLayout {
   int js;
@@ -42,17 +43,18 @@
   return by_lds > cap ? cap : (by_lds < 1 ? 1 : by_lds);
 }
 
-inline int front_rows_pick(int64_t n, int64_t h, int64_t w, int cin, size_t lds_fixed, int num_cu, int wg_cap, int forced = 0) {
+inline int front_rows_pick(int64_t n, int64_t h, int64_t w, int cin, size_t lds_fixed, int num_cu, int wg_cap, int forced = 0,
+                           size_t lds_max = kStatLdsMax, int wg_min = 2) {
   const int q = (int)(w / 4);
   int rmax = (int)(kFrontBandBytes / (32 * w));
   rmax = rmax > kFrontRows ? kFrontRows : rmax;
   rmax = rmax > h ? (int)h : rmax;
-  while (rmax >= 1 && lds_fixed + front_band_bytes(q, rmax, cin) > (size_t)kStatLdsMax) --rmax;
+  while (rmax >= 1 && lds_fixed + front_band_bytes(q, rmax, cin) > lds_max) --rmax;
   if (rmax < 1) return 0;
   if (forced > 0) return forced < rmax ? forced : rmax;
-  {
+  if (wg_min > 1) {
     int r2 = rmax;
-    while (r2 >= 1 && stat_wg_per_cu(lds_fixed + front_band_bytes(q, r2, cin), wg_cap) < 2) --r2;
+    while (r2 >= 1 && stat_wg_per_cu(lds_fixed + front_band_bytes(q, r2, cin), wg_cap) < wg_min) --r2;
     if (r2 >= 1) rmax = r2;
   }
   double best = 1e30;
diff --git a/quantization/mxnet_amd/csrc/fq_pwdw.hip b/quantization/mxnet_amd/csrc/fq_pwdw.hip
--- a/quantization/mxnet_amd/csrc/fq_pwdw.hip
+++ b/quantization/mxnet_amd/csrc/fq_pwdw.hip
@@ -467,31 +467,36 @@
   FrontLayout lay;
 };
 
-template <int KT, int FEPI = -1, bool FSIGNED = false>
-__global__ __launch_bounds__(kBlock, 3) void pw_stat_kernel(
+template <int KT, int FEPI = -1, bool FSIGNED = false, int NW = 4>
+__global__ __launch_bounds__(64 * NW, NW == 4 ? 3 : 1) void pw_stat_kernel(
     const float* __restrict__ x, const int8_t* __restrict__ wfrag, const float* __restrict__ wscale,
     const int* __restrict__ wsum, const float* __restrict__ bias, PwStatGeom g, const float* __restrict__ in_stat, int n,
     const float* __restrict__ in_thr, float levels, int lo_neg, float eps, float* __restrict__ cur_max_out,
     const float* __restrict__ bn_scale, const float* __restrict__ bn_shift, int act, float* __restrict__ stat_out,
     int8_t* __restrict__ x_codes_out, PwFrontArgs fa) {
   constexpr bool FRONT = FEPI >= 0;
-  static_assert(!FRONT || KT <= 4, "the front layer is built for up to four 32-channel slabs");
+  static_assert(NW == 4 ? (!FRONT || KT <= 4) : (NW == 8 && FRONT && KT == 8),
+                "the front layer: up to four 32-channel slabs on four wavefronts, eight slabs on eight");
+  constexpr int kThreads = 64 * NW;
+  constexpr bool kOneTable = NW != 4;
+  constexpr int kTables = kOneTable ? 1 : 4;
   extern __shared__ __attribute__((aligned(16))) unsigned char pst_smem[];
   v4i* ldsW = reinterpret_cast<v4i*>(pst_smem);
   int* c_zs = reinterpret_cast<int*>(pst_smem + (size_t)g.CT * KT * 1024);
   float* c_k = reinterpret_cast<float*>(c_zs + g.CT * 32);
   int* accs = reinterpret_cast<int*>(c_k + 4 * g.CT * 32);
-  float* dwk = reinterpret_cast<float*>(accs + 4 * g.CT * 128);
+  float* dwk = reinterpret_cast<float*>(accs + kTables * g.CT * 128);
   unsigned char* zbuf = reinterpret_cast<unsigned char*>(dwk + g.Cin * 12);
   const int lane = threadIdx.x & 63, wave = threadIdx.x >> 6;
   const int h = lane >> 5, i32 = lane & 31;
   const unsigned HW = (unsigned)g.HW, cols = (unsigned)g.cols;
-  const int64_t nwaves = (int64_t)gridDim.x * 4, wid = (int64_t)blockIdx.x * 4 + wave;
+  const int64_t nwaves = (int64_t)gridDim.x * NW, wid = (int64_t)blockIdx.x * NW + wave;
   const int64_t n_bands = FRONT ? (int64_t)(g.cols / g.HW) * fa.bands : 0;
   const int64_t t_begin = FRONT ? n_bands * blockIdx.x / gridDim.x : g.tiles * wid / nwaves;
   const int64_t t_end = FRONT ? n_bands * (blockIdx.x + 1) / gridDim.x : g.tiles * (wid + 1) / nwaves;
   const int pl = mfma_row_pixel(i32);
-  int* my = accs + (size_t)wave * g.CT * 128;
+  int* my = accs + (kOneTable ? (size_t)0 : (size_t)wave * g.CT * 128);
+  const int ct_lo = kOneTable ? wave : 0, ct_step = kOneTable ? NW : 1;
   constexpr int kSlots = 8;
   __shared__ unsigned k_stat[kSlots];
   if (threadIdx.x < kSlots) k_stat[threadIdx.x] = 0u;
@@ -542,12 +547,12 @@
   const unsigned nn_xor = fq_nonneg_xor(ubias);
   const bool wr_codes = x_codes_out != nullptr;
   const fq_rsrc rcodes = make_rsrc(x_codes_out, wr_codes ? (int64_t)(cols / HW) * 2 * KT * HW * 16 : 0);
-  for (int idx = threadIdx.x; idx < g.CT * KT * 64; idx += kBlock) {
+  for (int idx = threadIdx.x; idx < g.CT * KT * 64; idx += kThreads) {
     const int f = idx >> 6, ct = f / KT, kt = f - ct * KT;
     ldsW[idx] = *reinterpret_cast<const v4i*>(wfrag + (((int64_t)ct * g.KTS + kt) << 10) + ((idx & 63) << 4));
   }
   const int nchs = g.CT * 32;
-  for (int i = threadIdx.x; i < nchs; i += kBlock) {
+  for (int i = threadIdx.x; i < nchs; i += kThreads) {
     const bool okc = i < g.Cout;
     c_zs[i] = okc ? g.zoff * wsum[i] : 0;
     c_k[i] = okc ? wscale[i] : 0.0f;
@@ -556,7 +561,7 @@
     c_k[3 * nchs + i] = (okc && bn_scale != nullptr) ? bn_shift[i] : 0.0f;
   }
   if constexpr (FRONT)
-    for (int i = threadIdx.x; i < g.Cin; i += kBlock) {
+    for (int i = threadIdx.x; i < g.Cin; i += kThreads) {
 #pragma unroll
       for (int t = 0; t < 9; ++t) dwk[i * 12 + t] = fa.w[i * 9 + t];
       dwk[i * 12 + 9] = fa.bias != nullptr ? fa.bias[i] : 0.0f;
@@ -564,7 +569,7 @@
       dwk[i * 12 + 11] = fa.bn_scale != nullptr ? fa.bn_shift[i] : 0.0f;
     }
   auto reset = [&]() __attribute__((always_inline)) {
-    for (int ct = 0; ct < g.CT; ++ct) {
+    for (int ct = ct_lo; ct < g.CT; ct += ct_step) {
       my[ct * 128 + lane] = INT_MIN;
       my[ct * 128 + 64 + lane] = INT_MAX;
     }
@@ -574,7 +579,7 @@
   const bool has_bn = bn_scale != nullptr;
   auto flush = [&](unsigned smp) __attribute__((always_inline)) {
     float m = 0.0f;
-    for (int ct = 0; ct < g.CT; ++ct) {
+    for (int ct = ct_lo; ct < g.CT; ct += ct_step) {
       const int c = ct * 32 + i32;
       int hi = my[ct * 128 + lane], lo = my[ct * 128 + 64 + lane];
       const int ohi = __shfl_xor(hi, 32, 64), olo = __shfl_xor(lo, 32, 64);
@@ -629,33 +634,34 @@
     asm volatile("" : "+v"(f[0]), "+v"(f[1]), "+v"(f[2]), "+v"(f[3]));
     afrag[kt] = f;
   };
+  auto reduce_item = [&](int ct, int plo, int phi) __attribute__((always_inline)) {
+    const bool whole = plo <= 0 && phi >= 32;
+    v16i acc = {0, 0, 0, 0, 0, 0, 0, 0, 0, 0, 0, 0, 0, 0, 0, 0};
+#pragma unroll
+    for (int kt = 0; kt < KT; ++kt)
+      acc = __builtin_amdgcn_mfma_i32_32x32x32_i8(afrag[kt], ldsW[((ct * KT + kt) << 6) + lane], acc, 0, 0, 0);
+    int hi = INT_MIN, lo = INT_MAX;
+    if (whole) {
+#pragma unroll
+      for (int k = 0; k < 16; k += 2) {
+        hi = max(max(acc[k], acc[k + 1]), hi);
+        lo = min(min(acc[k], acc[k + 1]), lo);
+      }
+    } else {
+#pragma unroll
+      for (int k = 0; k < 16; ++k) {
+        const int p = 16 * h + k;
+        const bool in = p >= plo && p < phi;
+        hi = in && acc[k] > hi ? acc[k] : hi;
+        lo = in && acc[k] < lo ? acc[k] : lo;
+      }
+    }
+    atomicMax(&my[ct * 128 + lane], hi);
+    atomicMin(&my[ct * 128 + 64 + lane], lo);
+  };
   auto reduce_tile = [&](int plo, int phi) __attribute__((always_inline)) {
-    const bool whole = plo <= 0 && phi >= 32;
 #pragma unroll 1
-    for (int ct = 0; ct < g.CT; ++ct) {
-      v16i acc = {0, 0, 0, 0, 0, 0, 0, 0, 0, 0, 0, 0, 0, 0, 0, 0};
-#pragma unroll
-      for (int kt = 0; kt < KT; ++kt)
-        acc = __builtin_amdgcn_mfma_i32_32x32x32_i8(afrag[kt], ldsW[((ct * KT + kt) << 6) + lane], acc, 0, 0, 0);
-      int hi = INT_MIN, lo = INT_MAX;
-      if (whole) {
-#pragma unroll
-        for (int k = 0; k < 16; k += 2) {
-          hi = max(max(acc[k], acc[k + 1]), hi);
-          lo = min(min(acc[k], acc[k + 1]), lo);
-        }
-      } else {
-#pragma unroll
-        for (int k = 0; k < 16; ++k) {
-          const int p = 16 * h + k;
-          const bool in = p >= plo && p < phi;
-          hi = in && acc[k] > hi ? acc[k] : hi;
-          lo = in && acc[k] < lo ? acc[k] : lo;
-        }
-      }
-      atomicMax(&my[ct * 128 + lane], hi);
-      atomicMin(&my[ct * 128 + 64 + lane], lo);
-    }
+    for (int ct = 0; ct < g.CT; ++ct) reduce_item(ct, plo, phi);
   };
   unsigned cur = FRONT ? s_base : fast_div((unsigned)((t_begin < g.tiles ? t_begin : g.tiles - 1) * 32), g.hw);
   auto run_tile = [&](int64_t t, auto ph_c, auto nn_c) __attribute__((always_inline)) {
@@ -722,7 +728,7 @@
         flush(cur);
         cur = smp;
       }
-      for (int c0 = 0; c0 < g.Cin; c0 += 4 * fa.segs) {
+      for (int c0 = 0; c0 < g.Cin; c0 += NW * fa.segs) {
         const int c = front_channel(c0, wave, fa.segs, seg);
         const bool c_ok = seg < fa.segs && c < g.Cin;
         const int cc = c_ok ? c : 0;
@@ -782,7 +788,9 @@
       }
       __syncthreads();
       const int npix = Rb * W, ntile = (npix + 31) >> 5;
-      for (int tl = wave; tl < ntile; tl += 4) {
+      const int per_tile = kOneTable ? g.CT : 1, tl_step = NW / per_tile, ct_turn = NW - tl_step * per_tile;
+      int ct_it = kOneTable ? wave % per_tile : 0;
+      for (int tl = kOneTable ? wave / per_tile : wave; tl < ntile; tl += tl_step) {
         int pp = tl * 32 + pl;
         pp = pp < npix ? pp : npix - 1;
         const unsigned* zp = reinterpret_cast<const unsigned*>(zbuf + front_byte(fa.lay, g.Cin <= 16 ? 0 : 16 * h, pp));
@@ -792,12 +800,21 @@
 #pragma unroll
           for (int u = 0; u < 4; ++u) f[u] = (int)zp[(8 * kt + u) * fa.lay.pl];
           if (KT == 1 && g.Cin <= 16 && h == 1) f = zero_frag;
-          if (wr_codes)
+          if (wr_codes && ct_it == 0)
             buf_st_v4i(rcodes, ((smp * (unsigned)(2 * KT) + (unsigned)(2 * kt + h)) * HW + (unsigned)(r0 * W + pp)) * 16u, f);
           afrag[kt] = f;
         }
         const int valid = npix - tl * 32;
-        reduce_tile(0, valid < 32 ? valid : 32);
+        if constexpr (kOneTable) {
+          reduce_item(ct_it, 0, valid < 32 ? valid : 32);
+          ct_it += ct_turn;
+          if (ct_it >= per_tile) {
+            ct_it -= per_tile;
+            ++tl;
+          }
+        } else {
+          reduce_tile(0, valid < 32 ? valid : 32);
+        }
       }
       __syncthreads();
     }
@@ -830,7 +847,7 @@
   bool ok;
 };
 
-PwDwPlan pwdw_plan(int64_t n, int64_t cin, int64_t cout, int64_t h, int64_t w, int stride) {
+PwDwPlan pwdw_plan(int64_t n, int64_t cin, int64_t cout, int64_t h, int64_t w, int stride, bool ns = false) {
   PwDwPlan p;
   memset(&p, 0, sizeof(p));
   if (n <= 0 || cin <= 0 || cout <= 0 || h < 3 || w < 8 || (stride != 1 && stride != 2)) return p;
@@ -855,7 +872,8 @@
   const int rb_env = rb_e != nullptr ? atoi(rb_e) : 0;
   {
     const int waves = p.threads / 64;
-    int occ = (int)((160 * 1024) / (p.lds + 512));
+    const size_t lds_held = ns ? (size_t)ct * kt * 1024 + (size_t)cout * 13 * 4 : p.lds;
+    int occ = (int)((160 * 1024) / (lds_held + 512));
     const int by_regs = 8 / waves > 0 ? 8 / waves : 1;
     occ = occ < by_regs ? occ : by_regs;
     occ = occ < 1 ? 1 : occ;
@@ -883,7 +901,9 @@
 
 namespace fqi {
 
-static size_t pw_stat_lds(int kt, int ct) { return (size_t)ct * kt * 1024 + 5 * (size_t)ct * 32 * 4 + 4 * (size_t)ct * 128 * 4; }
+static size_t pw_stat_lds(int kt, int ct, int tables = 4) {
+  return (size_t)ct * kt * 1024 + 5 * (size_t)ct * 32 * 4 + (size_t)tables * ct * 128 * 4;
+}
 
 bool pw_stat_shape_ok(int64_t n, int64_t cin, int64_t cout, int64_t hw) {
   if (n <= 0 || cin <= 0 || cout <= 0 || hw < 32 || hw >= (1ll << 30) || n * hw >= (1ll << 31) - 512) return false;
@@ -893,16 +913,22 @@
 }
 
 constexpr int kFrontWgCap = 4;
+static bool pw_front_wide(int64_t cin) { return cin > 128; }
+static size_t pw_front_fixed_lds(int64_t cin, int64_t cout) {
+  return pw_stat_lds((int)((cin + 31) / 32), (int)((cout + 31) / 32), pw_front_wide(cin) ? 1 : 4) + (size_t)cin * 12 * 4;
+}
 
 static int pw_front_rows(int64_t n, int64_t cin, int64_t cout, int64_t h, int64_t w) {
   const char* e = getenv("FQ_PWSTAT_FRONT_ROWS");
   static const int wg_env = env_int("FQ_PWSTAT_WG_PER_CU", 0);
-  const size_t fixed = pw_stat_lds((int)((cin + 31) / 32), (int)((cout + 31) / 32)) + (size_t)cin * 12 * 4;
-  return front_rows_pick(n, h, w, (int)cin, fixed, num_cu(), wg_env > 0 ? wg_env : kFrontWgCap, e != nullptr ? atoi(e) : 0);
+  const int forced = e != nullptr ? atoi(e) : 0;
+  if (pw_front_wide(cin))
+    return front_rows_pick(n, h, w, (int)cin, pw_front_fixed_lds(cin, cout), num_cu(), 1, forced, (size_t)kStatLdsMaxWide, 1);
+  return front_rows_pick(n, h, w, (int)cin, pw_front_fixed_lds(cin, cout), num_cu(), wg_env > 0 ? wg_env : kFrontWgCap, forced);
 }
 
 bool pw_stat_front_shape_ok(int64_t n, int64_t cin, int64_t cout, int64_t h, int64_t w) {
-  if (h < 1 || w < 4 || w % 4 != 0 || w / 4 > 64 || !(cin == 16 || cin == 32 || cin == 64 || cin == 128) ||
+  if (h < 1 || w < 4 || w % 4 != 0 || w / 4 > 64 || !(cin == 16 || cin == 32 || cin == 64 || cin == 128 || cin == 256) ||
       !pw_stat_shape_ok(n, cin, cout, h * w))
     return false;
   return pw_front_rows(n, cin, cout, h, w) >= 1 && n * cin * ((w / 4 + 61) / 62) < (1ll << 31) - 1024;
@@ -922,16 +948,17 @@
     FQ_REQUIRE(fa.R >= 1, "fq_pwconv_i8_stat: no band of the front layer fits the LDS");
     fa.bands = (fa.H + fa.R - 1) / fa.R;
     fa.lay = front_layout(fa.Q, fa.R);
-    lds += (size_t)c.cin * 12 * 4 + front_band_bytes(fa.Q, fa.R, (int)c.cin);
+    lds = pw_front_fixed_lds(c.cin, c.cout) + front_band_bytes(fa.Q, fa.R, (int)c.cin);
   }
   PwStatGeom g;
   g.Cin = (int)c.cin; g.KTS = (int)(c.cin_pad / 32); g.Cout = (int)c.cout; g.CT = ct; g.HW = (int)c.hw;
   g.cols = c.n * c.hw; g.tiles = (g.cols + 31) / 32; g.zoff = c.zoff;
   g.hw = fast_div_for((unsigned)c.hw);
   if (int rc = pw_zero_stat(c)) return rc;
-  int per_cu = stat_wg_per_cu(lds, c.front != nullptr ? kFrontWgCap : 3);
+  const bool wide = c.front != nullptr && pw_front_wide(c.cin);
+  int per_cu = wide ? 1 : stat_wg_per_cu(lds, c.front != nullptr ? kFrontWgCap : 3);
   static const int wg_env = env_int("FQ_PWSTAT_WG_PER_CU", 0);
-  if (wg_env > 0) per_cu = wg_env;
+  if (wg_env > 0 && !wide) per_cu = wg_env;
   int64_t grid = (int64_t)num_cu() * per_cu;
   const int64_t need = c.front != nullptr ? c.n * fa.bands : (g.tiles + 3) / 4;
   if (grid > need) grid = need;
@@ -946,28 +973,32 @@
                        (const int*)c.wsum, c.bias, g, c.in_stat, (int)c.n, c.in_thr, c.levels, c.lo_neg, kEps,              \
                        c.out_current_max, c.bn_scale, c.bn_shift, c.act, c.stat_out, (int8_t*)c.x_codes_out, fa);          \
   } break;
-#define FQ_PST_FRONT(KT_, EPI_, SG_)                                                                                       \
+#define FQ_PST_FRONT(KT_, EPI_, SG_, NW_)                                                                                  \
   {                                                                                                                        \
-    static const bool attr_ok = hipFuncSetAttribute(reinterpret_cast<const void*>(&pw_stat_kernel<KT_, EPI_, SG_>),        \
-                                                    hipFuncAttributeMaxDynamicSharedMemorySize, 120 * 1024) == hipSuccess; \
+    static const bool attr_ok =                                                                                            \
+        hipFuncSetAttribute(reinterpret_cast<const void*>(&pw_stat_kernel<KT_, EPI_, SG_, NW_>),                           \
+                            hipFuncAttributeMaxDynamicSharedMemorySize, NW_ == 4 ? kStatLdsMax : kStatLdsMaxWide) == hipSuccess; \
     FQ_REQUIRE(attr_ok, "fq_pwconv_i8_stat: cannot raise the dynamic LDS limit");                                          \
-    hipLaunchKernelGGL((pw_stat_kernel<KT_, EPI_, SG_>), dim3((unsigned)grid), dim3(kBlock), lds, c.st, c.x, c.wcodes,     \
-                       c.wscale, (const int*)c.wsum, c.bias, g, c.in_stat, (int)c.n, c.in_thr, c.levels, c.lo_neg, kEps,   \
-                       c.out_current_max, c.bn_scale, c.bn_shift, c.act, c.stat_out, (int8_t*)c.x_codes_out, fa);          \
-  }
-#define FQ_PST_FRONT_S(KT_, EPI_)                                                                                          \
+    hipLaunchKernelGGL((pw_stat_kernel<KT_, EPI_, SG_, NW_>), dim3((unsigned)grid), dim3(64 * NW_), lds, c.st, c.x,        \
+                       c.wcodes, c.wscale, (const int*)c.wsum, c.bias, g, c.in_stat, (int)c.n, c.in_thr, c.levels,         \
+                       c.lo_neg, kEps, c.out_current_max, c.bn_scale, c.bn_shift, c.act, c.stat_out,                       \
+                       (int8_t*)c.x_codes_out, fa);                                                                        \
+  }
+#define FQ_PST_FRONT_S(KT_, EPI_, NW_)                                                                                     \
   {                                                                                                                        \
-    if (c.front->is_signed) FQ_PST_FRONT(KT_, EPI_, true) else FQ_PST_FRONT(KT_, EPI_, false)                              \
-  }
-#define FQ_PST_FRONT_E(KT_)                                                                                                \
+    if (c.front->is_signed) FQ_PST_FRONT(KT_, EPI_, true, NW_) else FQ_PST_FRONT(KT_, EPI_, false, NW_)                    \
+  }
+#define FQ_PST_FRONT_E(KT_, NW_)                                                                                           \
   {                                                                                                                        \
-    if (c.front->epi == kEpiBnRelu) FQ_PST_FRONT_S(KT_, kEpiBnRelu)                                                        \
-    else if (c.front->epi == kEpiBnRelu6) FQ_PST_FRONT_S(KT_, kEpiBnRelu6)                                                 \
-    else FQ_PST_FRONT_S(KT_, kEpiRuntime)                                                                                  \
+    if (c.front->epi == kEpiBnRelu) FQ_PST_FRONT_S(KT_, kEpiBnRelu, NW_)                                                   \
+    else if (c.front->epi == kEpiBnRelu6) FQ_PST_FRONT_S(KT_, kEpiBnRelu6, NW_)                                            \
+    else FQ_PST_FRONT_S(KT_, kEpiRuntime, NW_)                                                                             \
   }
   if (c.front != nullptr) {
-    FQ_REQUIRE(kt == 1 || kt == 2 || kt == 4, "fq_pwconv_i8_stat: a front layer needs cin <= 128");
-    if (kt == 1) FQ_PST_FRONT_E(1) else if (kt == 2) FQ_PST_FRONT_E(2) else FQ_PST_FRONT_E(4)
+    FQ_REQUIRE(kt == 1 || kt == 2 || kt == 4 || kt == 8, "fq_pwconv_i8_stat: a front layer needs cin <= 256");
+    FQ_REQUIRE(lds <= (size_t)(wide ? kStatLdsMaxWide : kStatLdsMax), "fq_pwconv_i8_stat: the band of the front layer does not fit the LDS");
+    if (kt == 1) FQ_PST_FRONT_E(1, 4) else if (kt == 2) FQ_PST_FRONT_E(2, 4) else if (kt == 4) FQ_PST_FRONT_E(4, 4)
+    else FQ_PST_FRONT_E(8, 8)
   } else {
     switch (kt) {
       FQ_PST_GO(1) FQ_PST_GO(2) FQ_PST_GO(4) FQ_PST_GO(8)
@@ -1036,7 +1067,7 @@
              "fq_pwdw_fused: unknown activation");
   FQ_REQUIRE(aligned16(wcodes) && (x_codes ? aligned16(x_codes) : aligned16(x)) && (ns || aligned16(y)),
              "fq_pwdw_fused: x (x_codes when given), wcodes and y must be 16-byte aligned");
-  const PwDwPlan p = pwdw_plan(n, cin, cout, h, w, dw_stride);
+  const PwDwPlan p = pwdw_plan(n, cin, cout, h, w, dw_stride, ns);
   FQ_REQUIRE(p.ok, "fq_pwdw_fused: shape not taken (n=%lld cin=%lld cout=%lld %lldx%lld stride %d): see fq_pwdw_fused_supported",
              (long long)n, (long long)cin, (long long)cout, (long long)h, (long long)w, dw_stride);
   hipStream_t st = (hipStream_t)stream;
diff --git a/quantization/mxnet_amd/ops.py b/quantization/mxnet_amd/ops.py
--- a/quantization/mxnet_amd/ops.py
+++ b/quantization/mxnet_amd/ops.py
@@ -672,6 +672,10 @@
     n, cin, h, w = (int(v) for v in xshape)
     lib = _lib_()
     return lib.fq_version() >= 102 and bool(lib.fq_pwdw_fused_supported(n, cin, int(cout), h, w, 1, 1))
+
+
+def pair_tail_supported():
+    return _lib_().fq_version() >= 103
 
 
 def pwdw_fused(x, wcodes, wscale, wsum, dw_w, pw_bias=None, in_stat=None, in_thr=None, width=8, flags=0, pw_bn_scale=None,
diff --git a/quantization/mxnet_amd/quantize/convert/convert_conv2d.py b/quantization/mxnet_amd/quantize/convert/convert_conv2d.py
--- a/quantization/mxnet_amd/quantize/convert/convert_conv2d.py
+++ b/quantization/mxnet_amd/quantize/convert/convert_conv2d.py
@@ -358,6 +358,19 @@
     return one.expand(*shape)
 
 
+def _beyond_the_pairs_that_pay(xshape):
+    from .. import fuse as _fuse
+    return xshape[2] * xshape[3] < _fuse.RECOMPUTE_MIN_PIXELS or xshape[1] > _fuse.RECOMPUTE_MAX_CIN
+
+
+def _tail_takes(xshape):
+    from .. import fuse as _fuse
+    level = int(_fuse.PAIR_TAIL)
+    if not level or xshape[1] > _fuse.TAIL_MAX_CIN or xshape[2] * xshape[3] < _fuse.TAIL_MIN_PIXELS:
+        return False
+    return (level >= 2 or ops.in_flight()) and ops.pair_tail_supported()
+
+
 def recompute_target(block, fz, x, plan, c16_in):
     from .. import fuse as _fuse
     nxt = fz.get("pair_dw")
@@ -374,7 +387,7 @@
     if any(_hooked(b) for b in (block, nxt, fz.get("bn"), fz.get("act_block"))):
         return None
     t = x._t
-    if t.dim() != 4 or t.shape[2] * t.shape[3] < _fuse.RECOMPUTE_MIN_PIXELS or t.shape[1] > _fuse.RECOMPUTE_MAX_CIN:
+    if t.dim() != 4 or (_beyond_the_pairs_that_pay(t.shape) and not _tail_takes(t.shape)):
         return None
     if not ops.pwdw_supported(tuple(t.shape), block._kwargs["num_filter"], nxt._kwargs["stride"][0]):
         return None
@@ -402,7 +415,8 @@
     from .. import fuse as _fuse
     if d.get("x_codes") is None or fz.get("front_pw") is None:
         return None
-    nxt = front_target(block, fz, x, dict(in_stat=x._fq_stat, width=width), level=_fuse.PAIR_CHAIN)
+    tail = _beyond_the_pairs_that_pay(d["x"].shape) or _beyond_the_pairs_that_pay(x._t.shape)
+    nxt = front_target(block, fz, x, dict(in_stat=x._fq_stat, width=width), level=_fuse.PAIR_TAIL if tail else _fuse.PAIR_CHAIN)
     if nxt is None or not ops.pwdw_chain_supported(tuple(d["x"].shape), block._kwargs["num_filter"]):
         return None
     return nxt
diff --git a/quantization/mxnet_amd/quantize/fuse.py b/quantization/mxnet_amd/quantize/fuse.py
--- a/quantization/mxnet_amd/quantize/fuse.py
+++ b/quantization/mxnet_amd/quantize/fuse.py
@@ -131,6 +131,8 @@
 PAIR_CODES = _os.environ.get("FQ_PWDW_CODES", "1") != "0"
 PAIR_FRONT = int(_os.environ.get("FQ_PWDW_FRONT", "1"))
 PAIR_CHAIN = int(_os.environ.get("FQ_PWDW_CHAIN", "1"))
+PAIR_TAIL = int(_os.environ.get("FQ_PWDW_TAIL", "0"))
+TAIL_MAX_CIN, TAIL_MIN_PIXELS = 256, 784
 SUBSAMPLE = _os.environ.get("FQ_SUBSAMPLE", "1") != "0"
 GAP_FUSE = _os.environ.get("FQ_GAP_FUSE", "1") != "0"
 SHORTCUT_FUSE = _os.environ.get("FQ_SHORTCUT_FUSE", "1") != "0"
```

Result: slower. 161,400 (-1.6%).
